# jwh97nn/AnyRef

Measured on AMD Instinct MI355X. Metric: images/sec (1024^2, 7B LLM+ViT-L+SAM-H), higher is better.
Workload: dtype bf16 (LLaMA / CLIP) + f16 (SAM encoder); 1 GPU; C2: LLaVA-7B + CLIP ViT-L/14 + SAM-H refer-seg forward, 1024x1024, S=320 prompt, 10 new tokens, KV cache; batch_per_gpu=1, global_batch=1, parallelism=dp1, weights=random-init N(0,0.02^2) rounded to bf16

## Files before the change

### anyref_amd/_lib.py

```python
from __future__ import annotations

import ctypes as C
import os

import torch

HERE = os.path.dirname(os.path.abspath(__file__))
LIB_PATH = os.path.join(HERE, "libanyref_hip.so")

ABI_VERSION = 2
F32, BF16, F16 = 0, 1, 2
MODE_PARITY, MODE_PERF, MODE_PERF_FP8W, MODE_PARITY16, MODE_PERF_F16, MODE_PARITY16_F16 = 0, 1, 2, 3, 4, 5
MODE_PERF_INT4W = 6


class AnyrefConfig(C.Structure):
    _fields_ = [
        ("abi_version", C.c_int32), ("mode", C.c_int32),
        ("clip_image", C.c_int32), ("clip_patch", C.c_int32), ("clip_dim", C.c_int32),
        ("clip_heads", C.c_int32), ("clip_layers_run", C.c_int32), ("clip_mlp", C.c_int32),
        ("clip_eps", C.c_float),
        ("llm_vocab", C.c_int32), ("llm_dim", C.c_int32), ("llm_heads", C.c_int32),
        ("llm_layers", C.c_int32), ("llm_mlp", C.c_int32), ("llm_max_seq", C.c_int32),
        ("llm_rms_eps", C.c_float), ("llm_rope_theta", C.c_float),
# ... 22 lines not shown
                                   "norm_out", "slabs_out")] +
                [(n, _L) for n in ("sA", "sW", "sC", "sR", "sBias")] +
                [(n, C.c_int32) for n in ("M", "N", "K", "lda", "ldw", "ldc", "ldr", "norm_ld", "act", "c_f32",
                                          "swiglu_pairs", "slabs", "max_wg", "batch")] +
                [("alpha", _F), ("norm_eps", _F), ("norm_done", C.c_int32)])


class NormEx(C.Structure):
    _fields_ = ([(n, _P) for n in ("x", "gain", "bias", "y", "row_map", "fill_dst", "fill_rows", "fill_bias")] +
                [(n, C.c_int32) for n in ("M", "D", "ldx", "ldy", "rms", "y_f32", "act", "fill_ld", "fill_n", "fill_N",
                                          "fill_fallback")] +
                [("eps", _F), ("fill_done", C.c_int32)])


class AttnEx(C.Structure):
    _fields_ = ([(n, _P) for n in ("q", "k", "v", "o", "q_pos0", "kv_len", "q_len", "rel_h", "rel_w", "rel_p",
                                   "rel_tab_h", "rel_tab_w")] +
                [(n, _L) for n in ("q_bs", "q_rs", "q_hs", "k_bs", "k_rs", "k_hs", "v_bs", "v_rs", "v_hs", "o_bs", "o_rs",
                                   "o_hs", "rel_hs")] +
                [(n, C.c_int32) for n in ("B", "H", "Sq", "Sk", "hd", "causal", "kh", "kw", "rel_ld", "rel_tab_ld",
                                          "max_wg")] +
                [("scale", _F)])

SYMBOLS = {
    "anyref_create": (_I, [C.POINTER(AnyrefConfig), _I, C.POINTER(_P)]),
    "anyref_destroy": (None, [_P]),
    "anyref_last_error": (C.c_char_p, [_P]),
    "anyref_set_weight": (_I, [_P, C.c_char_p, _P, _I, _I, C.POINTER(_L), _I]),
    "anyref_finalize": (_I, [_P]),
    "anyref_generate": (_I, [_P, _P, _P, _P, _P, _P, _I, _I, _P, _P, _I, _P, _P, _I, _I, _P, _P, _P, _P, _L, _P,
                             _P, _P]),
    "anyref_forward_teacher": (_I, [_P, _P, _P, _P, _P, _P, _I, _I, _P, _P, _I, _P, _P, _P, _P, _P, _L, _P, _P,
                                    _P, _P]),
    "anyref_encode_images": (_I, [_P, _P, _P, _I, _P, _P]),
    "anyref_sam_encode": (_I, [_P, _P, _P, _I, _P]),
    "anyref_mask_decode": (_I, [_P, _P, _P, _P, _I, _P, _P, _P, _P, _P]),
    "anyref_llm_forward": (_I, [_P, _P, _P, _P, _I, _I, _P, _P, _P, _P]),
    "anyref_project_audio": (_I, [_P, _P, _P, _I, _P]),
    "anyref_audio_encode": (_I, [_P, _P, _P, _I, _P]),
    "anyref_seg_tail": (_I, [_P, _P, _P, _P, _P, _P, _I, _I, _I, _P, _I, _P, _P, _P, _P, _P, _L, _P, _P]),
    "anyref_set_seg_range": (_I, [_P, _I, _I]),
    "anyref_set_overlap": (_I, [_P, _I]),
    "anyref_set_early_tail": (_I, [_P, _I]),
    "anyref_set_extra_event": (_I, [_P, _P]),
    "anyref_set_graphs": (_I, [_P, _I]),
    "anyref_set_side_share": (_I, [_P, _I, _I]),
    "anyref_profile_enable": (_I, [_P, _I]),
    "anyref_profile_config": (_I, [_P, C.c_char_p, _I]),
    "anyref_profile_collect": (_I, [_P]),
    "anyref_profile_calibrate": (_I, [_P, _P, C.POINTER(C.c_double)]),
    "anyref_profile_read": (_I, [_P, _I, C.c_char_p, _I, C.POINTER(C.c_double), C.POINTER(_L),
                                C.POINTER(C.c_double), C.POINTER(C.c_double)]),
    "anyref_stamps_enable": (_I, [_P, _I]),
    "anyref_stamps_collect": (_I, [_P, C.POINTER(_L)]),
    "anyref_stamps_dropped": (_I, [_P, C.POINTER(_L)]),
    "anyref_stamps_read": (_I, [_P, _L, C.c_char_p, _I, C.POINTER(C.c_double), C.POINTER(C.c_double),
                               C.POINTER(C.c_double), C.POINTER(_I)]),
    "anyref_stamps_spread": (_I, [_P, _L, C.POINTER(C.c_double), C.POINTER(C.c_double), C.POINTER(C.c_double)]),
    "anyref_device_bytes": (_L, [_P]),
    "anyref_mode_name": (C.c_char_p, [_P]),
    "anyref_inexact_weights": (_I, [_P, C.POINTER(_L)]),
    "anyref_op_gemm": (_I, [_I, _P, _P, _P, _P, _P, _P, _P, _I, _I, _I, _I, _I]),
    "anyref_op_gemm_fp8": (_I, [_P, _P, _P, _P, _P, _P, _P, _I, _I, _I, _I, _I]),
    "anyref_op_quant_fp8": (_I, [_P, _P, _I, _I, _P, _P]),
    "anyref_op_gemv_fp8": (_I, [_P, _P, _P, _F, _P, _P, _P, _P, _P, _P, _I, _I, _I]),
    "anyref_op_quant_int4": (_I, [_P, _P, _I, _I, _P, _P]),
    "anyref_op_dequant_int4": (_I, [_P, _P, _P, _I, _I, _P]),
    "anyref_op_gemm_int4": (_I, [_P, _P, _P, _P, _P, _P, _P, _I, _I, _I, _I, _I, _I]),
    "anyref_op_gemv_int4": (_I, [_P, _P, _P, _F, _P, _P, _P, _P, _P, _P, _I, _I, _I]),
    "anyref_op_iou_counts": (_I, [_P, _P, _P, _I, _L, _P]),
    "anyref_op_avs_counts": (_I, [_P, _P, _P, _I, _L, _P, _I, _F, _P, _P]),
    "anyref_op_sam_preprocess": (_I, [_P, _P, _I, _I, _I, C.POINTER(C.c_float), C.POINTER(C.c_float), _P]),
    "anyref_op_pil_resample_u8": (_I, [_P, _P, _I, _I, _I, _P, _P, _I, _I, _P, _P, _I, _P, _P, _I]),
    "anyref_op_pool_ref_tokens": (_I, [_P, _P, _I, _I, _I, _I, _P]),
    "anyref_op_kaldi_fbank": (_I, [_P, _P, _I, _I, _I, _I, _I, C.c_float, _P, _I, _P, _P, _I, C.c_float, C.c_float, _P]),
    "anyref_op_clip_finish": (_I, [_P, _P, _I, _I, _I, _I, _I, _I, _I, C.POINTER(C.c_float), C.POINTER(C.c_float), _P]),
    "anyref_op_gemv": (_I, [_I, _P, _P, _P, _F, _P, _P, _P, _P, _P, _I, _I, _I, _I]),
    "anyref_op_gemv_xn": (_I, [_I, _P, _P, _P, _F, _P, _P, _P, _P, _P, _I, _I, _I, _I, _P, _P, _I]),
    "anyref_op_split_roundtrip": (_I, [_I, _P, _P, _P, _P, _I, _I]),
    "anyref_op_rope_table": (_I, [_I, _I, _F, _P]),
    "anyref_op_decode_attn": (_I, [_I, _P, _P, _I, _I, _I, _P, _P, _P, _P, _I, _F, _P, _P, _I]),
    "anyref_op_rope_cache": (_I, [_I, _P, _P, _P, _P, _I, _I, _I, _I, _P, _P, _P, _P, _P, _P, _I, _P]),
    "anyref_op_argmax": (_I, [_P, _P, _I, _I, _I, _P, _P, _P, _I, _I, _I, _P, _P, _P]),
    "anyref_op_norm": (_I, [_I, _P, _P, _P, _P, _P, _I, _I, _F, _I]),
    "anyref_op_attention": (_I, [_I, _P, _P, _P, _P, _P, _I, _I, _I, _I, _I, _F, _I, _P, _P, _P, _I, _I]),
    "anyref_op_attention_tab": (_I, [_I, _P, _P, _P, _P, _P, _I, _I, _I, _I, _F, _P, _P, _I, _I, _I]),
    "anyref_op_gemm_gather": (_I, [_I, _P, _P, _P, _P, _P, _P, _P, _I, _I, _I, _I]),
    "anyref_op_attention_relp": (_I, [_I, _P, _P, _P, _P, _P, _I, _I, _I, _I, _F, _P, _I, _I, _I]),
    "anyref_op_rel_pos": (_I, [_I, _P, _P, _P, _P, _I, _I, _I, _I, _P, _P]),
    "anyref_op_postprocess": (_I, [_P, _P, _I, _I, _I, _I, _I, _I, _I, _I, _P]),
    "anyref_op_last_error": (C.c_char_p, []),
    "anyref_op_gemm_ex": (_I, [_I, _P, C.POINTER(GemmEx)]),
    "anyref_op_norm_ex": (_I, [_I, _P, C.POINTER(NormEx)]),
    "anyref_op_attention_ex": (_I, [_I, _P, C.POINTER(AttnEx)]),
    "anyref_op_last_tags": (C.c_char_p, []),
}

_lib = None


def load() -> C.CDLL:
    global _lib
    if _lib is not None:
        return _lib
    if not os.path.exists(LIB_PATH):
        raise RuntimeError(
            f"{LIB_PATH} not found: build the HIP backend first "
            "(`python -c 'import __graft_entry__ as g; g.build()'` or `make -C anyref_amd/csrc`). "
            "anyref_amd has no CPU fallback.")
    lib = C.CDLL(LIB_PATH)
    for name, (res, args) in SYMBOLS.items():
        fn = getattr(lib, name)
        fn.restype = res
        fn.argtypes = args
    _lib = lib
    return lib
```

### anyref_amd/csrc/common.h

```cpp
#pragma once
#include <hip/hip_runtime.h>
#include <stdint.h>
#include <atomic>
#include <stdio.h>
#include <stdexcept>

namespace anyref {

struct bf16 {
  uint16_t x;
};

__host__ __device__ inline float bf2f(bf16 h) {
  uint32_t u = ((uint32_t)h.x) << 16;
  return __builtin_bit_cast(float, u);
}
__device__ inline bf16 f2bf(float f) {
  __bf16 h = (__bf16)f;
  bf16 r;
  r.x = __builtin_bit_cast(uint16_t, h);
  return r;
}
inline bf16 f2bf_host(float f) {
  uint32_t u = __builtin_bit_cast(uint32_t, f);
// ... 207 lines not shown
  }
};
template <>
struct Vec16<float> {
  static constexpr int N = 4;
  static __device__ inline void unpack(const uint4v& v, float* f) {
#pragma unroll
    for (int i = 0; i < 4; ++i) {
      const uint32_t u = v[i];
      f[i] = __builtin_bit_cast(float, u);
    }
  }
};

typedef __attribute__((ext_vector_type(4))) short short4v_;
typedef __attribute__((ext_vector_type(8))) _Float16 half8v;
typedef __attribute__((ext_vector_type(4))) _Float16 half4v;
template <typename T>
__device__ __forceinline__ float4v mfma_16x16x32(short8 a, short8 b, float4v c) {
  if constexpr (is_half16<T>::value)
    return __builtin_amdgcn_mfma_f32_16x16x32_f16(__builtin_bit_cast(half8v, a), __builtin_bit_cast(half8v, b), c, 0, 0, 0);
  else
    return __builtin_amdgcn_mfma_f32_16x16x32_bf16(a, b, c, 0, 0, 0);
}
template <typename T>
__device__ __forceinline__ float4v mfma_16x16x16(short4v_ a, short4v_ b, float4v c) {
  if constexpr (is_half16<T>::value)
    return __builtin_amdgcn_mfma_f32_16x16x16f16(__builtin_bit_cast(half4v, a), __builtin_bit_cast(half4v, b), c, 0, 0, 0);
  else
    return __builtin_amdgcn_mfma_f32_16x16x16bf16_1k(a, b, c, 0, 0, 0);
}

typedef float float2v __attribute__((ext_vector_type(2)));
__device__ inline void unpack_fp8x16(const uint4v& v, float* f) {
#pragma unroll
  for (int i = 0; i < 4; ++i) {
    const int w = (int)v[i];
    const float2v lo = __builtin_amdgcn_cvt_pk_f32_fp8(w, false);
    const float2v hi = __builtin_amdgcn_cvt_pk_f32_fp8(w, true);
    f[4 * i] = lo[0]; f[4 * i + 1] = lo[1]; f[4 * i + 2] = hi[0]; f[4 * i + 3] = hi[1];
  }
}
constexpr float FP8_E4M3_MAX = 448.f;

enum Act : int { ACT_NONE = 0, ACT_RELU = 1, ACT_GELU = 2, ACT_QUICK_GELU = 3, ACT_SILU = 4 };

__device__ inline float apply_act(float v, int act) {
  switch (act) {
    case ACT_RELU:
      return v > 0.f ? v : 0.f;
    case ACT_GELU:
      return 0.5f * v * (1.f + erff(v * 0.70710678118654752f));
    case ACT_QUICK_GELU:
      return v / (1.f + __expf(-1.702f * v));
    case ACT_SILU:
      return v / (1.f + __expf(-v));
    default:
      return v;
  }
}

__device__ inline float gelu_fast(float v) {
  const float x = fabsf(v) * 0.70710678118654752f;
  const float t = __builtin_amdgcn_rcpf(fmaf(0.3275911f, x, 1.f));
  float p = fmaf(1.061405429f, t, -1.453152027f);
  p = fmaf(p, t, 1.421413741f);
  p = fmaf(p, t, -0.284496736f);
  p = fmaf(p, t, 0.254829592f);
  const float e = 1.f - p * t * __expf(-x * x);
  return 0.5f * v * (1.f + copysignf(e, v));
}

__device__ inline float wave_sum(float v) {
#pragma unroll
  for (int o = 32; o > 0; o >>= 1) v += __shfl_xor(v, o, 64);
  return v;
}
__device__ inline float wave_max(float v) {
#pragma unroll
  for (int o = 32; o > 0; o >>= 1) v = fmaxf(v, __shfl_xor(v, o, 64));
  return v;
}

#define HIP_TRY(expr)                                                                   \
  do {                                                                                  \
    hipError_t _e = (expr);                                                             \
    if (_e != hipSuccess) {                                                             \
      char _b[512];                                                                     \
      snprintf(_b, sizeof(_b), "%s failed: %s (%s:%d)", #expr, hipGetErrorString(_e), __FILE__, \
               __LINE__);                                                               \
      throw std::runtime_error(_b);                                                     \
    }                                                                                   \
  } while (0)

struct KernelAttrOnce {
  std::atomic<uint64_t> done[4] = {};
};
inline void ensure_dyn_lds(KernelAttrOnce& st, const void* kernel, int bytes) {
  int dev = 0;
  HIP_TRY(hipGetDevice(&dev));
  std::atomic<uint64_t>& word = st.done[(dev >> 6) & 3];
  const uint64_t bit = 1ull << (dev & 63);
  if (word.load(std::memory_order_acquire) & bit) return;
  HIP_TRY(hipFuncSetAttribute(kernel, hipFuncAttributeMaxDynamicSharedMemorySize, bytes));
  word.fetch_or(bit, std::memory_order_release);
}
inline int device_cus() {
  static std::atomic<int> cache[256] = {};
  int dev = 0;
  HIP_TRY(hipGetDevice(&dev));
  std::atomic<int>& c = cache[dev & 255];
  int v = c.load(std::memory_order_relaxed);
  if (!v) {
    HIP_TRY(hipDeviceGetAttribute(&v, hipDeviceAttributeMultiprocessorCount, dev));
    c.store(v, std::memory_order_relaxed);
  }
  return v;
}

__host__ __device__ inline int cdiv(int a, int b) { return (a + b - 1) / b; }
inline int64_t cdiv64(int64_t a, int64_t b) { return (a + b - 1) / b; }
inline int round_up(int a, int b) { return cdiv(a, b) * b; }

}
```

### anyref_amd/csrc/gemv.hip

```cpp
#include <cstdlib>
#include <stdexcept>
#include <type_traits>

#include "gemv_common.h"

namespace anyref {

#ifndef ANYREF_GEMV_NO_DOT2
#define ANYREF_GEMV_NO_DOT2 0
#endif
constexpr bool NO_DOT2 = ANYREF_GEMV_NO_DOT2;
template <typename T, int NB, bool DUAL, int XPT, bool W8 = false, bool PAIR = false>
__global__ __launch_bounds__(512) void gemv_kernel(GemvArgs a, int b0, int nb) {
  static_assert(!W8 || std::is_same<T, bf16>::value, "fp8 weights go with bf16 activations");
  using WE = typename split_term<T>::type;
  using XE = std::conditional_t<is_split<T>::value, float, T>;
  using WT = std::conditional_t<W8, uint8_t, WE>;
  constexpr int VN = W8 ? 16 : Vec16<WE>::N;
  constexpr int R = DUAL ? 1 : 2;
  constexpr int RW = 2;
  constexpr int UNR = 4;
  constexpr bool DOT2 = (std::is_same<T, bf16>::value || is_half16<T>::value) && !W8 && !NO_DOT2;
  extern __shared__ __attribute__((aligned(16))) char smem[];
  XE* xs = reinterpret_cast<XE*>(smem);
  __shared__ float red[NB][8];
  __shared__ float red2[2][4][2][NB];
  const int tid = threadIdx.x, lane = tid & 63, wave = tid >> 6;
  const int K = a.K;
  __shared__ unsigned long long st_t[2];
  __shared__ unsigned st_cnt;
  const unsigned long long t_begin = gemv_stamp_begin(a.stamp, st_t, st_cnt, tid);

  const WT* __restrict__ W = reinterpret_cast<const WT*>(a.W);
  const WT* __restrict__ W2 = reinterpret_cast<const WT*>(a.W2);
  const int ldw = a.ldw > 0 ? a.ldw : K;
  constexpr int CH = 64 * VN * UNR;
  const GemvWork<R, PAIR> wk(gridDim.x, blockIdx.x, wave, a.N, cdiv(K, CH));
  const int items = wk.items;
  uint4v wcur[UNR][RW], wnxt[UNR][RW];
  auto load_item = [&](int t, uint4v (&w)[UNR][RW]) {
    const auto it = wk.item(t);
    const int n0 = it.g * R;
#pragma unroll
    for (int u = 0; u < UNR; ++u) {
      const int k = it.live ? it.c * CH + u * 64 * VN + lane * VN : K;
#pragma unroll
      for (int r = 0; r < R; ++r) {
        const int n = n0 + r < a.N ? n0 + r : a.N - 1;
        w[u][r] = k < K ? __builtin_nontemporal_load(reinterpret_cast<const uint4v*>(W + (int64_t)n * ldw + k))
                        : uint4v{0, 0, 0, 0};
      }
      if (DUAL)
        w[u][RW - 1] = k < K ? __builtin_nontemporal_load(reinterpret_cast<const uint4v*>(W2 + (int64_t)n0 * ldw + k))
                             : uint4v{0, 0, 0, 0};
    }
  };
  if (!a.gain) {
    constexpr int XV = (XPT + 3) / 4;
    float4v xv[NB][XV];
#pragma unroll
    for (int b = 0; b < NB; ++b) {
      const float* x = a.x + (int64_t)(b0 + (b < nb ? b : 0)) * a.ldx;
#pragma unroll
      for (int i = 0; i < XV; ++i) {
        const int k = (tid + i * 512) * 4;
        xv[b][i] = (b < nb && k < K) ? *reinterpret_cast<const float4v*>(x + k) : float4v{0.f, 0.f, 0.f, 0.f};
      }
    }
    if (items > 0) load_item(0, wcur);
#pragma unroll
    for (int b = 0; b < NB; ++b) {
      if (b >= nb) continue;
#pragma unroll
      for (int i = 0; i < XV; ++i) {
        const int k = (tid + i * 512) * 4;
        if (k < K) store4_from_f32<XE>(&xs[b * K + k], xv[b][i][0], xv[b][i][1], xv[b][i][2], xv[b][i][3]);
      }
    }
  } else {
    constexpr int XV = (XPT + 3) / 4;
    GemvNormStage<NB, XV> st;
    st.load(a, b0, nb, tid);
    if (items > 0) load_item(0, wcur);
    float scale[NB];
    st.scales(a, red, lane, wave, scale);
#pragma unroll
    for (int b = 0; b < NB; ++b) {
      if (b >= nb) continue;
#pragma unroll
      for (int i = 0; i < XV; ++i) {
        const int k = (tid + i * 512) * 4;
        if (k < K) {
          const float4v v = st.xr[b][i] * scale[b] * st.gr[i];
          store4_from_f32<XE>(&xs[b * K + k], v[0], v[1], v[2], v[3]);
          gemv_store_xn(a, b0 + b, k, v);
        }
      }
    }
  }
  __syncthreads();

  float acc[RW][NB];
#pragma unroll
  for (int r = 0; r < RW; ++r)
#pragma unroll
    for (int b = 0; b < NB; ++b) acc[r][b] = 0.f;
  for (int t = 0; t < items; ++t) {
    if (t + 1 < items) load_item(t + 1, wnxt);
    const auto it = wk.item(t);
#pragma unroll
    for (int u = 0; u < UNR; ++u) {
      const int k = it.live ? it.c * CH + u * 64 * VN + lane * VN : K;
      if (k < K) {
        if constexpr (DOT2) {
          typedef __attribute__((ext_vector_type(2))) __bf16 bf16x2;
          typedef __attribute__((ext_vector_type(2))) _Float16 f16x2;
          uint4v xv[NB];
#pragma unroll
          for (int b = 0; b < NB; ++b)
            xv[b] = b < nb ? *reinterpret_cast<const uint4v*>(&xs[b * K + k]) : uint4v{0, 0, 0, 0};
#pragma unroll
          for (int r = 0; r < RW; ++r)
#pragma unroll
            for (int b = 0; b < NB; ++b)
#pragma unroll
              for (int j = 0; j < 4; ++j) {
                const uint32_t wj = wcur[u][r][j], xj = xv[b][j];
                if constexpr (is_half16<T>::value)
                  acc[r][b] = __builtin_amdgcn_fdot2(__builtin_bit_cast(f16x2, wj), __builtin_bit_cast(f16x2, xj), acc[r][b],
                                                     false);
                else
                  acc[r][b] = __builtin_amdgcn_fdot2_f32_bf16(__builtin_bit_cast(bf16x2, wj), __builtin_bit_cast(bf16x2, xj),
                                                              acc[r][b], false);
              }
        } else {
        float xf[NB][VN];
#pragma unroll
        for (int b = 0; b < NB; ++b) {
          if (b < nb) {
            constexpr int XV = Vec16<XE>::N;
#pragma unroll
            for (int h = 0; h < VN / XV; ++h) {
              const uint4v xv = *reinterpret_cast<const uint4v*>(&xs[b * K + k + h * XV]);
              Vec16<XE>::unpack(xv, &xf[b][h * XV]);
            }
          } else {
#pragma unroll
            for (int i = 0; i < VN; ++i) xf[b][i] = 0.f;
          }
        }
#pragma unroll
        for (int r = 0; r < RW; ++r) {
          float wf[VN];
          if constexpr (W8) unpack_fp8x16(wcur[u][r], wf);
          else Vec16<WE>::unpack(wcur[u][r], wf);
#pragma unroll
          for (int b = 0; b < NB; ++b)
#pragma unroll
            for (int i = 0; i < VN; ++i) acc[r][b] = fmaf(wf[i], xf[b][i], acc[r][b]);
        }
        }
      }
    }
    if (it.last) gemv_finish_group<NB, R, DUAL, W8, PAIR>(a, acc, red2, it.g, it.pass, wk.half, lane, wave, b0, nb);
    if (t + 1 < items) {
#pragma unroll
      for (int u = 0; u < UNR; ++u)
#pragma unroll
        for (int r = 0; r < RW; ++r) wcur[u][r] = wnxt[u][r];
    }
  }
  gemv_stamp_end(a.stamp, st_t, st_cnt, t_begin, lane);
}

template <bool W8, bool DUAL, int XV>
__global__ __launch_bounds__(512) void gemv_rows8_kernel(GemvArgs a, int b0, int nb, int kh0, int rs) {
  typedef __attribute__((ext_vector_type(2))) __bf16 bf16x2;
  constexpr int NB = 8, UNR = 8;
  constexpr int EPL = W8 ? 16 : 8;
  constexpr int SEG = 16 * EPL;
  constexpr int CH = UNR * SEG;
  using WT = std::conditional_t<W8, uint8_t, bf16>;
  extern __shared__ __attribute__((aligned(16))) char smem[];
  __shared__ float red[NB][8];
  const int tid = threadIdx.x, lane = tid & 63, wave = tid >> 6;
  const int j = lane & 3, q = lane >> 2;
  const int K = a.K;
  const int ldw = a.ldw > 0 ? a.ldw : K;
  const WT* __restrict__ W = reinterpret_cast<const WT*>(a.W);
  const WT* __restrict__ W2 = reinterpret_cast<const WT*>(a.W2);
  constexpr int R = DUAL ? 2 : 4;
  const int ngroups = cdiv(a.N, R);
  const int nwaves = gridDim.x * 8, gw = blockIdx.x * 8 + wave;
  const int my_groups = gw < ngroups ? (ngroups - gw + nwaves - 1) / nwaves : 0;
  const int nkh = kh0 < K ? 2 : 1;
  const int nch0 = cdiv(kh0, CH), nch1 = nkh == 2 ? cdiv(K - kh0, CH) : 0;
  const int items0 = my_groups * nch0, items = items0 + my_groups * nch1;
  const int pl = rs > 0 ? (rs - 64) / 2 : 0;
  uint4v w0[UNR], w1[UNR], w2[UNR];
  auto item_pos = [&](int t, int& g, int& kbeg, int& kend) __attribute__((always_inline)) {
    int gi, c;
    if (t < items0) {
      gi = t / nch0; c = t - gi * nch0;
      kbeg = c * CH; kend = kh0;
    } else {
      const int t1 = t - items0;
      gi = t1 / nch1; c = t1 - gi * nch1;
      kbeg = kh0 + c * CH; kend = K;
    }
    g = gw + gi * nwaves;
  };
  auto load_item = [&](int t, uint4v (&w)[UNR]) __attribute__((always_inline)) {
    int g, kbeg, kend;
    item_pos(t, g, kbeg, kend);
    const int jl = lane >> 4, ql = lane & 15;
    int n = DUAL ? g * 2 + (jl & 1) : g * 4 + jl;
    n = n < a.N ? n : a.N - 1;
    const WT* row = ((DUAL && jl >= 2) ? W2 : W) + (int64_t)n * ldw;
#pragma unroll
    for (int u = 0; u < UNR; ++u) {
      const int k = kbeg + u * SEG + ql * EPL;
      w[u] = k < kend ? __builtin_nontemporal_load(reinterpret_cast<const uint4v*>(row + k)) : uint4v{0, 0, 0, 0};
    }
  };
  auto xpos = [&](int b, int kl) __attribute__((always_inline)) {
    if constexpr (W8) return b * rs + ((kl >> 3) & 1) * pl + (kl >> 4) * 16 + (kl & 7) * 2;
    else return b * rs + kl * 2;
  };
  auto first_chunks = [&]() __attribute__((always_inline)) {
    if (items > 0) load_item(0, w0);
    if (items > 1) load_item(1, w1);
  };
  float scale[NB];
#pragma unroll
  for (int b = 0; b < NB; ++b) scale[b] = 1.f;
  if (a.gain) {
    GemvNormStage<NB, XV> st;
    st.load(a, b0, nb, tid);
    first_chunks();
    st.scales(a, red, lane, wave, scale);
#pragma unroll
    for (int b = 0; b < NB; ++b) {
#pragma unroll
      for (int i = 0; i < XV; ++i) {
        const int k = (tid + i * 512) * 4;
        if (k < K) {
          const float4v v = st.xr[b][i] * scale[b] * st.gr[i];
          store4_from_f32<bf16>(reinterpret_cast<bf16*>(smem + xpos(b, k)), v[0], v[1], v[2], v[3]);
          gemv_store_xn(a, b0 + b, k, v, b < nb);
        }
      }
    }
  }
  auto stage_plain = [&](int kbase, int klen, bool then_weights) __attribute__((always_inline)) {
// ... 119 lines not shown
    run(items0, items);
  }
}

static bool gemv_rows8_launch(const GemvArgs& a, int b0, int nb, hipStream_t s) {
  static const bool off = getenv("ANYREF_GEMV_ROWS8") && atoi(getenv("ANYREF_GEMV_ROWS8")) == 0;
  if (off) return false;
  const bool w8 = a.w_fp8 != 0, dual = a.W2 != nullptr;
  const int epl = w8 ? 16 : 8, ch = 8 * 16 * epl;
  const int ldw = a.ldw > 0 ? a.ldw : a.K;
  const size_t wsz = w8 ? 1 : 2;
  if (a.K % epl || (ldw * wsz) % 16 || ((uintptr_t)a.W & 15) || (dual && ((uintptr_t)a.W2 & 15)) || a.K % 4) return false;
  constexpr int KH_MAX = 9472;
  int kh0 = a.K;
  if (a.gain) {
    if (a.K > 6144) return false;
  } else if (a.K > KH_MAX) {
    kh0 = cdiv(cdiv(a.K, 2), ch) * ch;
    if (kh0 > KH_MAX || kh0 >= a.K) return false;
    if (cdiv(a.N, dual ? 2 : 4) > 256 * 8) return false;
  }
  const int rs = cdiv(kh0 * 2, 256) * 256 + 64;
  const size_t lds = (size_t)8 * rs;
  const int grid = 256;
  const double wbytes = (double)a.N * a.K * wsz * (dual ? 2 : 1) + (double)nb * (a.K + a.N) * 4;
  char tag[48];
  snprintf(tag, sizeof(tag), "gemv_rows8_%s%s", w8 ? "fp8w" : "bf16", dual ? "_swiglu" : "");
  ProfScope prof(tag, 2.0 * nb * a.N * (double)a.K * (dual ? 2 : 1), wbytes, s);
  auto launch = [&](auto w8_t, auto dual_t, auto xv_t) {
    gemv_launch<&gemv_rows8_kernel<decltype(w8_t)::value, decltype(dual_t)::value, decltype(xv_t)::value>, 152 * 1024>(
        grid, lds, s, a, b0, nb, kh0, rs);
  };
  using TT = std::true_type;
  using FF = std::false_type;
  using X2 = std::integral_constant<int, 2>;
  using X3 = std::integral_constant<int, 3>;
  auto by_xv = [&](auto w8_t, auto dual_t) {
    if (a.gain && a.K > 4096) launch(w8_t, dual_t, X3());
    else launch(w8_t, dual_t, X2());
  };
  if (w8) {
    if (dual) by_xv(TT(), TT());
    else by_xv(TT(), FF());
  } else {
    if (dual) by_xv(FF(), TT());
    else by_xv(FF(), FF());
  }
  return true;
}

template <typename T, int NB>
static void gemv_dispatch(const GemvArgs& a, int b0, int nb, hipStream_t s) {
  const size_t lds = (size_t)NB * a.K * (is_split<T>::value ? 4 : sizeof(T));
  const double wsz = a.w_fp8 ? 1.0 : (is_split<T>::value ? 2.0 : (double)sizeof(T));
  const double wbytes = (double)a.N * a.K * wsz * (a.W2 ? 2 : 1) + (double)nb * (a.K + a.N) * 4;
  const char* kind = a.w_fp8 ? "fp8w" : (is_split<T>::value ? (is_half16<typename split_term<T>::type>::value ? "sp16h" : "sp16") : is_half16<T>::value ? "f16" : sizeof(T) == 2 ? "bf16" : "f32");
  gemv_dispatch_pass("gemv", kind, a, lds, wbytes, nb, s, [&](auto xpt_t, auto dual_t, auto pair_t, const GemvArgs& g, int grid) {
    constexpr int XPT = decltype(xpt_t)::value;
    constexpr bool DUAL = decltype(dual_t)::value, PAIR = decltype(pair_t)::value;
    if constexpr (std::is_same<T, bf16>::value) {
      if (g.w_fp8) {
        gemv_launch<&gemv_kernel<T, NB, DUAL, XPT, true, PAIR>>(grid, lds, s, g, b0, nb);
        return;
      }
    }
    gemv_launch<&gemv_kernel<T, NB, DUAL, XPT, false, PAIR>>(grid, lds, s, g, b0, nb);
  });
}

template <typename T>
void launch_gemv(const GemvArgs& a, hipStream_t s) {
  if (a.w_int4) {
    if (!std::is_same<T, bf16>::value) throw std::runtime_error("gemv: int4 weights need the bf16 mode");
    launch_gemv_int4(a, s);
    return;
  }
  const int VN = a.w_fp8 ? 16 : Vec16<typename split_term<T>::type>::N;
  if (a.K % VN || ((uintptr_t)a.W & 15)) throw std::runtime_error("gemv: K must be a multiple of 16 bytes");
  if (a.w_fp8 && (!std::is_same<T, bf16>::value || !a.wscale || (a.W2 && !a.wscale2)))
    throw std::runtime_error("gemv: fp8 weights need the bf16 mode and per-row scales");
  if (((uintptr_t)a.x & 15) || a.ldx % 4 || a.K % 4 || (a.gain && ((uintptr_t)a.gain & 15)) ||
      (a.xn_out && (((uintptr_t)a.xn_out & 15) || a.xn_ld % 4)))
    throw std::runtime_error("gemv: x / gain / xn_out rows must be 16-byte aligned");
  int b0 = 0;
  if constexpr (std::is_same<T, bf16>::value) {
    while (a.B - b0 > 4) {
      const int n8 = a.B - b0 < 8 ? a.B - b0 : 8;
      if (!gemv_rows8_launch(a, b0, n8, s)) break;
      b0 += n8;
    }
  }
  gemv_passes<sizeof(T) == 2 ? 4 : 2>(b0, a.B, [&](auto nb_t, int p0, int nb) { gemv_dispatch<T, decltype(nb_t)::value>(a, p0, nb, s); });
}
template void launch_gemv<float>(const GemvArgs&, hipStream_t);

void launch_gemv_skinny_f32(const GemvArgs& a, hipStream_t s) {
  if (a.B < 1 || a.B > 8 || a.K > 4096 || a.K % 4 || a.W2 || a.w_fp8 || a.gain || ((uintptr_t)a.W & 15) ||
      ((uintptr_t)a.x & 15) || a.ldx % 4)
    throw std::runtime_error("gemv_skinny_f32: 1..8 rows, K <= 4096, K % 4 == 0, 16-byte aligned rows");
  const int ngroups = cdiv(a.N, 2);
  const int grid = ngroups >= 2048 ? 512 : cdiv(ngroups, 4);
  auto go = [&](auto nb_tag) {
    constexpr int NB = decltype(nb_tag)::value;
    ProfScope prof("gemv_f32_skinny", 2.0 * a.B * a.N * (double)a.K, (double)a.N * a.K * 4 + (double)a.B * (a.K + a.N) * 4,
                   s);
    gemv_launch<&gemv_kernel<float, NB, false, 8, false, true>>(grid, (size_t)NB * a.K * sizeof(float), s, a, 0, a.B);
  };
  if (a.B == 1) go(std::integral_constant<int, 1>());
  else if (a.B == 2) go(std::integral_constant<int, 2>());
  else if (a.B <= 4) go(std::integral_constant<int, 4>());
  else go(std::integral_constant<int, 8>());
}
template void launch_gemv<bf16>(const GemvArgs&, hipStream_t);
template void launch_gemv<sp16>(const GemvArgs&, hipStream_t);
template void launch_gemv<sp16h>(const GemvArgs&, hipStream_t);
template void launch_gemv<f16>(const GemvArgs&, hipStream_t);

}
```

### anyref_amd/csrc/gemv_common.h

```cpp
#pragma once
#include <cstdlib>
#include <stdexcept>
#include <string>
#include <type_traits>

#include "kernels.h"

namespace anyref {

template <int R, bool PAIR>
struct GemvWork {
  int ngroups, nch, unit, nunits, half, nchp, items;
  __device__ __forceinline__ GemvWork(unsigned grid, unsigned block, int wave, int N, int nch_) {
    const int nwaves = grid * 8, gw = block * 8 + wave;
    ngroups = cdiv(N, R);
    nch = nch_;
    unit = PAIR ? gw >> 1 : gw;
    nunits = PAIR ? nwaves >> 1 : nwaves;
    half = PAIR ? (gw & 1) : 0;
    nchp = PAIR ? (nch + 1) >> 1 : nch;
    const int my_groups = PAIR ? cdiv(ngroups, nunits) : (gw < ngroups ? (ngroups - gw + nwaves - 1) / nwaves : 0);
    items = my_groups * nchp;
  }
  struct Item {
    int pass, g, c;
    bool live, last;
  };
  __device__ __forceinline__ Item item(int t) const {
    const int pass = t / nchp, ci = t % nchp;
    const int g = unit + pass * nunits, c = PAIR ? 2 * ci + half : ci;
    return {pass, g, c, !PAIR || (g < ngroups && c < nch), ci == nchp - 1};
  }
};

template <int NB, int XV>
struct GemvNormStage {
  float4v xr[NB][XV], gr[XV];
  __device__ __forceinline__ void load_gain(const GemvArgs& a, int tid) {
#pragma unroll
    for (int i = 0; i < XV; ++i) {
      const int k = (tid + i * 512) * 4;
      gr[i] = k < a.K ? *reinterpret_cast<const float4v*>(a.gain + k) : float4v{1.f, 1.f, 1.f, 1.f};
    }
  }
  __device__ __forceinline__ void load_x(const GemvArgs& a, int b0, int nb, int tid) {
#pragma unroll
    for (int b = 0; b < NB; ++b) {
      const float* x = a.x + (int64_t)(b0 + (b < nb ? b : 0)) * a.ldx;
#pragma unroll
      for (int i = 0; i < XV; ++i) {
        const int k = (tid + i * 512) * 4;
        xr[b][i] = (b < nb && k < a.K) ? *reinterpret_cast<const float4v*>(x + k) : float4v{0.f, 0.f, 0.f, 0.f};
      }
    }
  }
  __device__ __forceinline__ void load(const GemvArgs& a, int b0, int nb, int tid) {
    load_gain(a, tid);
    load_x(a, b0, nb, tid);
  }
  __device__ __forceinline__ void scales(const GemvArgs& a, float (&red)[NB][8], int lane, int wave, float (&scale)[NB]) const {
#pragma unroll
    for (int b = 0; b < NB; ++b) {
      float ss = 0.f;
#pragma unroll
      for (int i = 0; i < XV; ++i)
#pragma unroll
        for (int e = 0; e < 4; ++e) ss += xr[b][i][e] * xr[b][i][e];
      ss = wave_sum(ss);
      if (lane == 0) red[b][wave] = ss;
    }
    __syncthreads();
#pragma unroll
    for (int b = 0; b < NB; ++b) {
      float tot = 0.f;
#pragma unroll
      for (int w = 0; w < 8; ++w) tot += red[b][w];
      scale[b] = rsqrtf(tot / (float)a.K + a.eps);
    }
  }
};
__device__ __forceinline__ void gemv_store_xn(const GemvArgs& a, int row, int k, float4v v, bool also = true) {
  if (a.xn_out && blockIdx.x == 0 && also)
    *reinterpret_cast<float4v*>(a.xn_out + (int64_t)(a.xn_row_map ? a.xn_row_map[row] : row) * a.xn_ld + k) = v;
}

template <bool DUAL, bool W8>
__device__ __forceinline__ void gemv_epilogue(const GemvArgs& a, float v, float v2, int n, int row) {
  if constexpr (W8) {
    v *= a.wscale[(int64_t)n * a.ws_stride];
    if (DUAL) v2 *= a.wscale2[(int64_t)n * a.ws_stride];
  }
  if (a.bias) v += a.bias[n];
  if (DUAL)
    v = apply_act(v, ACT_SILU) * v2;
  else
    v = apply_act(v, a.act);
  const int64_t o = (int64_t)row * a.ldy + n;
  if (a.resid) v += a.resid[o];
  a.y[o] = v;
}

template <int NB, int R, bool DUAL, bool W8, bool PAIR>
__device__ __forceinline__ void gemv_finish_group(const GemvArgs& a, float (&acc)[2][NB], float (&red2)[2][4][2][NB], int g,
                                                  int pass, int half, int lane, int wave, int b0, int nb) {
  constexpr int RW = 2;
  const int n0 = g * R;
#pragma unroll
  for (int r = 0; r < RW; ++r)
#pragma unroll
    for (int b = 0; b < NB; ++b) acc[r][b] = wave_sum(acc[r][b]);
  if constexpr (PAIR) {
    const int buf = pass & 1;
    if (half == 1 && lane == 0) {
#pragma unroll
      for (int r = 0; r < RW; ++r)
#pragma unroll
        for (int b = 0; b < NB; ++b) red2[buf][wave >> 1][r][b] = acc[r][b];
    }
    __syncthreads();
    if (half == 0) {
#pragma unroll
      for (int r = 0; r < RW; ++r)
#pragma unroll
        for (int b = 0; b < NB; ++b) acc[r][b] += red2[buf][wave >> 1][r][b];
    }
  }
  if (lane < R * NB && half == 0) {
    const int r = lane / NB, b = lane % NB, n = n0 + r;
    float v = 0.f, v2 = 0.f;
#pragma unroll
    for (int rr = 0; rr < R; ++rr)
#pragma unroll
      for (int bb = 0; bb < NB; ++bb)
        if (lane == rr * NB + bb) {
          v = acc[rr][bb];
          v2 = DUAL ? acc[RW - 1][bb] : 0.f;
        }
    if (n < a.N && b < nb) gemv_epilogue<DUAL, W8>(a, v, v2, n, b0 + b);
  }
#pragma unroll
  for (int r = 0; r < RW; ++r)
#pragma unroll
    for (int b = 0; b < NB; ++b) acc[r][b] = 0.f;
}

__device__ __forceinline__ unsigned long long gemv_stamp_begin(const StampArgs& st, unsigned long long (&st_t)[2],
                                                               unsigned& st_cnt, int tid) {
  unsigned long long t_begin = 0;
  if (st.base) {
    t_begin = wall_clock64();
    if (tid == 0) {
      st_t[0] = ~0ull;
      st_t[1] = 0;
      st_cnt = 0;
    }
  }
  return t_begin;
}
__device__ __forceinline__ void gemv_stamp_end(const StampArgs& st, unsigned long long (&st_t)[2], unsigned& st_cnt,
                                               unsigned long long t_begin, int lane) {
  if (st.base && lane == 0) {
    atomicMin(&st_t[0], t_begin);
    atomicMax(&st_t[1], (unsigned long long)wall_clock64());
    if (atomicAdd(&st_cnt, 1u) == 7u) {
      const int e = *st.epoch;
      if (e < st.max_epoch) {
        unsigned long long* p = st.base + (size_t)e * st.stride + (size_t)blockIdx.x * 2;
        p[0] = st_t[0];
        p[1] = st_t[1];
      }
    }
  }
}

inline bool gemv_pair_knob() {
  static const bool p = !(getenv("ANYREF_GEMV_PAIR") && atoi(getenv("ANYREF_GEMV_PAIR")) == 0);
  return p;
}
inline int gemv_grid_knob() {
  static const int g = getenv("ANYREF_GEMV_GRID") ? atoi(getenv("ANYREF_GEMV_GRID")) : 0;
  return g;
}

struct GemvPlan {
  int grid;
  bool pair;
};
inline GemvPlan gemv_plan(const GemvArgs& a, size_t lds) {
  const int grid_rule = 256 * (lds > 76 * 1024 ? 1 : 2);
  int grid = grid_rule;
  if (a.grid > 0 && a.grid < grid) grid = a.grid;
  if (gemv_grid_knob() > 0) grid = gemv_grid_knob();
  const bool pair = gemv_pair_knob() && cdiv(a.N, a.W2 ? 1 : 2) * 2 <= (gemv_grid_knob() > 0 ? grid : grid_rule) * 8;
  return {grid, pair};
}

template <auto KERN, int LDS_MAX = 150 * 1024, typename... Args>
inline void gemv_launch(int grid, size_t lds, hipStream_t s, Args... args) {
  static KernelAttrOnce once;
  ensure_dyn_lds(once, reinterpret_cast<const void*>(KERN), LDS_MAX);
  hipLaunchKernelGGL(KERN, dim3(grid), dim3(512), lds, s, args...);
}

template <typename Launch>
inline void gemv_dispatch_pass(const char* name, const char* kind, const GemvArgs& a_in, size_t lds, double wbytes, int nb,
                               hipStream_t s, Launch&& launch) {
  GemvArgs a = a_in;
  if (lds > 150 * 1024) throw std::runtime_error(std::string(name) + ": K too large for the LDS activation stage");
  const GemvPlan p = gemv_plan(a, lds);
  auto go = [&](auto xpt_t) {
    char tag[40];
    snprintf(tag, sizeof(tag), "gemv_%s%s_x%d", kind, a.W2 ? "_swiglu" : "", decltype(xpt_t)::value);
    ProfScope prof(tag, 2.0 * nb * a.N * (double)a.K * (a.W2 ? 2 : 1), wbytes, s);
    if (g_stamp && g_stamp->on) a.stamp = g_stamp->slot(tag, wbytes, p.grid);
    using TT = std::true_type;
    using FF = std::false_type;
    if (a.W2) {
      if (p.pair) launch(xpt_t, TT(), TT(), a, p.grid);
      else launch(xpt_t, TT(), FF(), a, p.grid);
    } else {
      if (p.pair) launch(xpt_t, FF(), TT(), a, p.grid);
      else launch(xpt_t, FF(), FF(), a, p.grid);
    }
  };
  if (a.K <= 512 * 8)
    go(std::integral_constant<int, 8>());
  else if (a.K <= 512 * 24)
    go(std::integral_constant<int, 24>());
  else if (a.K <= 512 * 32)
    go(std::integral_constant<int, 32>());
  else
    throw std::runtime_error(std::string(name) + ": K > 16384 not supported");
}

template <int NBMAX, typename Pass>
inline void gemv_passes(int b0, int B, Pass&& pass) {
  while (b0 < B) {
    const int left = B - b0, nb = left < NBMAX ? left : NBMAX;
    if (nb == 1)
      pass(std::integral_constant<int, 1>(), b0, nb);
    else if (nb == 2)
      pass(std::integral_constant<int, 2>(), b0, nb);
    else
      pass(std::integral_constant<int, NBMAX>(), b0, nb);
    b0 += nb;
  }
}

}
```

### anyref_amd/csrc/gemv_int4.hip

```cpp
#include <cstdlib>
#include <stdexcept>
#include <type_traits>

#include "gemv_common.h"

namespace anyref {

constexpr int I4_GROUP = 128;
constexpr int I4_BLOCK = 32;
constexpr float I4_BIAS = 136.f;

__global__ __launch_bounds__(256) void quant_int4_rows_kernel(const float* __restrict__ src, int lds, int K,
                                                              uint8_t* __restrict__ q, int ldq, bf16* __restrict__ scale,
                                                              int lds_scale, unsigned long long* __restrict__ inexact) {
  const int n = blockIdx.x, tid = threadIdx.x;
  const float* row = src + (int64_t)n * lds;
  uint32_t* out = reinterpret_cast<uint32_t*>(q + (int64_t)n * ldq);
  const int G = cdiv(K, I4_GROUP);
  unsigned changed = 0;
  for (int g0 = 0; g0 < G; g0 += 16) {
    const int g = g0 + (tid >> 4), k0 = g * I4_GROUP + (tid & 15) * 8;
    float w[8];
    float amax = 0.f;
#pragma unroll
// ... 76 lines not shown
  typedef __attribute__((ext_vector_type(2))) __bf16 bf16x2;
  constexpr int R = DUAL ? 1 : 2;
  constexpr int RW = 2;
  constexpr int UNR = XPT == 8 ? (PAIR ? 1 : 2) : XPT == 24 ? 3 : 4;
  constexpr int CHB = 64 * UNR;
  extern __shared__ __attribute__((aligned(16))) char smem[];
  __shared__ float red[NB][8];
  __shared__ float red2[2][4][2][NB];
  const int tid = threadIdx.x, lane = tid & 63, wave = tid >> 6;
  const int K = a.K, KB = cdiv(K, I4_BLOCK);
  const int row_bytes = KB * 64;
  float* xsum = reinterpret_cast<float*>(smem + (size_t)NB * row_bytes);
  __shared__ unsigned long long st_t[2];
  __shared__ unsigned st_cnt;
  const unsigned long long t_begin = gemv_stamp_begin(a.stamp, st_t, st_cnt, tid);

  const uint8_t* __restrict__ W = reinterpret_cast<const uint8_t*>(a.W);
  const uint8_t* __restrict__ W2 = reinterpret_cast<const uint8_t*>(a.W2);
  const uint16_t* __restrict__ S = reinterpret_cast<const uint16_t*>(a.gscale);
  const uint16_t* __restrict__ S2 = reinterpret_cast<const uint16_t*>(a.gscale2);
  const int ldw = a.ldw, lgs = a.ld_gscale;
  const GemvWork<R, PAIR> wk(gridDim.x, blockIdx.x, wave, a.N, cdiv(KB, CHB));
  const int items = wk.items;
  uint4v wcur[UNR][RW], wnxt[UNR][RW];
  uint32_t scur[UNR][RW], snxt[UNR][RW];
  auto load_item = [&](int t, uint4v (&w)[UNR][RW], uint32_t (&sc)[UNR][RW]) {
    const auto it = wk.item(t);
    const int n0 = it.g * R;
#pragma unroll
    for (int u = 0; u < UNR; ++u) {
      const int blk = it.live ? it.c * CHB + u * 64 + lane : KB;
#pragma unroll
      for (int r = 0; r < R; ++r) {
        const int n = n0 + r < a.N ? n0 + r : a.N - 1;
        w[u][r] = blk < KB ? __builtin_nontemporal_load(reinterpret_cast<const uint4v*>(W + (int64_t)n * ldw + blk * 16))
                           : uint4v{0, 0, 0, 0};
        sc[u][r] = blk < KB ? (uint32_t)S[(int64_t)n * lgs + (blk >> 2)] : 0u;
      }
      if (DUAL) {
        w[u][RW - 1] = blk < KB ? __builtin_nontemporal_load(reinterpret_cast<const uint4v*>(W2 + (int64_t)n0 * ldw + blk * 16))
                                : uint4v{0, 0, 0, 0};
        sc[u][RW - 1] = blk < KB ? (uint32_t)S2[(int64_t)n0 * lgs + (blk >> 2)] : 0u;
      }
    }
  };
  {
    constexpr int XV = (XPT + 3) / 4;
    GemvNormStage<NB, XV> st;
    if (a.gain) st.load_gain(a, tid);
    st.load_x(a, b0, nb, tid);
    if (items > 0) load_item(0, wcur, scur);
    float scale[NB];
#pragma unroll
    for (int b = 0; b < NB; ++b) scale[b] = 1.f;
    if (a.gain) st.scales(a, red, lane, wave, scale);
#pragma unroll
    for (int b = 0; b < NB; ++b) {
#pragma unroll
      for (int i = 0; i < XV; ++i) {
        const int k = (tid + i * 512) * 4;
        const float4v v = a.gain ? st.xr[b][i] * scale[b] * st.gr[i] : st.xr[b][i];
        const bf16 h0 = f2bf(v[0]), h1 = f2bf(v[1]), h2 = f2bf(v[2]), h3 = f2bf(v[3]);
        float sum = (bf2f(h0) + bf2f(h1)) + (bf2f(h2) + bf2f(h3));
        sum += __shfl_xor(sum, 1, 64);
        sum += __shfl_xor(sum, 2, 64);
        sum += __shfl_xor(sum, 4, 64);
        const int blk = k >> 5, in = k & 31;
        if (b < nb && blk < KB) {
          char* p = smem + (size_t)b * row_bytes + (size_t)(in >> 3) * (KB * 16) + blk * 16 + (in & 7) * 2;
          *reinterpret_cast<uint2v*>(p) = uint2v{(uint32_t)h0.x | ((uint32_t)h1.x << 16), (uint32_t)h2.x | ((uint32_t)h3.x << 16)};
          if ((tid & 7) == 0) xsum[b * KB + blk] = sum;
          if (a.gain) gemv_store_xn(a, b0 + b, k, v, k < K);
        }
      }
    }
  }
  __syncthreads();

  float acc[RW][NB];
#pragma unroll
  for (int r = 0; r < RW; ++r)
#pragma unroll
    for (int b = 0; b < NB; ++b) acc[r][b] = 0.f;
  for (int t = 0; t < items; ++t) {
    if (t + 1 < items) load_item(t + 1, wnxt, snxt);
    const auto it = wk.item(t);
#pragma unroll
    for (int u = 0; u < UNR; ++u) {
      const int blk = it.live ? it.c * CHB + u * 64 + lane : KB;
      if (blk < KB) {
        uint32_t pr[RW][16];
#pragma unroll
        for (int r = 0; r < RW; ++r)
#pragma unroll
          for (int d = 0; d < 4; ++d) {
            const uint32_t wd = wcur[u][r][d];
#pragma unroll
            for (int j = 0; j < 4; ++j) pr[r][d * 4 + j] = ((wd >> (4 * j)) & 0x000F000Fu) | 0x43004300u;
          }
        float sf[RW];
#pragma unroll
        for (int r = 0; r < RW; ++r) sf[r] = __builtin_bit_cast(float, scur[u][r] << 16);
#pragma unroll
        for (int b = 0; b < NB; ++b) {
          if (b >= nb) continue;
          const char* xb = smem + (size_t)b * row_bytes + blk * 16;
          uint4v xv[4];
#pragma unroll
          for (int d = 0; d < 4; ++d) xv[d] = *reinterpret_cast<const uint4v*>(xb + (size_t)d * (KB * 16));
          const float t0 = -I4_BIAS * xsum[b * KB + blk];
#pragma unroll
          for (int r = 0; r < RW; ++r) {
            float tt = t0;
#pragma unroll
            for (int d = 0; d < 4; ++d)
#pragma unroll
              for (int j = 0; j < 4; ++j) {
                const uint32_t xj = xv[d][j], pj = pr[r][d * 4 + j];
                tt = __builtin_amdgcn_fdot2_f32_bf16(__builtin_bit_cast(bf16x2, pj), __builtin_bit_cast(bf16x2, xj), tt, false);
              }
            acc[r][b] = fmaf(sf[r], tt, acc[r][b]);
          }
        }
      }
    }
    if (it.last) gemv_finish_group<NB, R, DUAL, false, PAIR>(a, acc, red2, it.g, it.pass, wk.half, lane, wave, b0, nb);
    if (t + 1 < items) {
#pragma unroll
      for (int u = 0; u < UNR; ++u)
#pragma unroll
        for (int r = 0; r < RW; ++r) {
          wcur[u][r] = wnxt[u][r];
          scur[u][r] = snxt[u][r];
        }
    }
  }
  gemv_stamp_end(a.stamp, st_t, st_cnt, t_begin, lane);
}

template <int NB>
static void gemv_int4_dispatch(const GemvArgs& a, int b0, int nb, hipStream_t s) {
  const int KB = cdiv(a.K, I4_BLOCK), G = cdiv(a.K, I4_GROUP);
  const size_t lds = (size_t)NB * KB * (64 + 4);
  const double wbytes = (double)a.N * ((double)a.K * 0.5 + G * 2.0) * (a.W2 ? 2 : 1) + (double)nb * (a.K + a.N) * 4;
  gemv_dispatch_pass("gemv_int4", "int4w", a, lds, wbytes, nb, s, [&](auto xpt_t, auto dual_t, auto pair_t, const GemvArgs& g, int grid) {
    gemv_launch<&gemv_int4_kernel<NB, decltype(dual_t)::value, decltype(xpt_t)::value, decltype(pair_t)::value>>(grid, lds, s, g, b0, nb);
  });
}

void launch_gemv_int4(const GemvArgs& a, hipStream_t s) {
  const int G = cdiv(a.K, I4_GROUP);
  if (a.K % 16 || ((uintptr_t)a.W & 15) || ((uintptr_t)a.W2 & 15) || a.ldw % 16 || a.ldw < G * 64)
    throw std::runtime_error("gemv_int4: K must be a multiple of 16 and nibble rows 16-byte aligned, whole groups long");
  if (!a.gscale || (a.W2 && !a.gscale2) || a.ld_gscale < G) throw std::runtime_error("gemv_int4: group scales missing");
  if (((uintptr_t)a.x & 15) || a.ldx % 4 || (a.gain && ((uintptr_t)a.gain & 15)) ||
      (a.xn_out && (((uintptr_t)a.xn_out & 15) || a.xn_ld % 4)))
    throw std::runtime_error("gemv_int4: x / gain / xn_out rows must be 16-byte aligned");
  gemv_passes<4>(0, a.B, [&](auto nb_t, int b0, int nb) { gemv_int4_dispatch<decltype(nb_t)::value>(a, b0, nb, s); });
}

}
```

### anyref_amd/csrc/kernels.h

```cpp
#pragma once
#include <cstdlib>
#include <map>
#include <string>
#include <utility>
#include <vector>

#include "common.h"

namespace anyref {

struct ProfStat {
  double ms = 0;
  int64_t count = 0;
  double flops = 0, bytes = 0;
};
class Profiler {
 public:
  ~Profiler();
  bool begin(const char* tag, double flops, double bytes, hipStream_t s);
  void end(hipStream_t s);
  void collect();
  void reset();
  void calibrate(hipStream_t s);
  double null_ms = 0.0;
// ... 56 lines not shown
  size_t cap_used_ = 0;
  int64_t dropped_ = 0;
  std::vector<Rec> eager_;
  std::map<int, std::vector<Rec>> graphs_;
  std::vector<int> epoch_keys_;
};
extern thread_local Stamper* g_stamp;
struct ProfScope {
  hipStream_t s;
  bool active;
  ProfScope(const char* tag, double flops, double bytes, hipStream_t st) : s(st), active(g_prof && g_prof->on) {
    if (active) active = g_prof->begin(tag, flops, bytes, s);
  }
  ~ProfScope() {
    if (active) g_prof->end(s);
  }
};

struct GemmArgs {
  const void* A = nullptr;
  const void* W = nullptr;
  const float* bias = nullptr;
  void* C = nullptr;
  const float* resid = nullptr;
  const int* row_map = nullptr;
  const int* a_row_map = nullptr;
  int M = 0, N = 0, K = 0;
  int lda = 0, ldw = 0, ldc = 0, ldr = 0;
  int act = ACT_NONE;
  int c_f32 = 0;
  float alpha = 1.f;
  int order = 3;
  int swiglu_pairs = 0;
  int w_fp8 = 0;
  const float* col_scale = nullptr;
  int w_int4 = 0;
  const void* gscale = nullptr;
  int ld_gscale = 0;
  int group_m = 0;
  int max_wg = 0;
  int vec_ok = 0;
  const float* norm_gain = nullptr;
  void* norm_out = nullptr;
  int norm_ld = 0;
  float norm_eps = 0.f;
  const float* norm_bias = nullptr;
  float* slabs_out = nullptr;
  int slabs = 0;
  bool* norm_done = nullptr;
  int batch = 1;
  int64_t sA = 0, sW = 0, sC = 0, sR = 0, sBias = 0;
};
template <typename T>
void launch_gemm(const GemmArgs& a, hipStream_t s);
void gemm_reserve_workspace(hipStream_t s, size_t bytes);
void gemm_release_workspace(hipStream_t s);
void attn_release_workspace(hipStream_t s);

struct GemvArgs {
  const float* x = nullptr;
  const float* gain = nullptr;
  float eps = 1e-6f;
  const void* W = nullptr;
  const void* W2 = nullptr;
  const float* bias = nullptr;
  float* y = nullptr;
  const float* resid = nullptr;
  int B = 1, N = 0, K = 0, ldx = 0, ldy = 0;
  int act = ACT_NONE;
  int ldw = 0;
  int w_fp8 = 0;
  const float* wscale = nullptr;
  const float* wscale2 = nullptr;
  int ws_stride = 1;
  int w_int4 = 0;
  const void* gscale = nullptr;
  const void* gscale2 = nullptr;
  int ld_gscale = 0;
  float* xn_out = nullptr;
  const int* xn_row_map = nullptr;
  int xn_ld = 0;
  StampArgs stamp;
  int grid = 0;
};
template <typename T>
void launch_gemv(const GemvArgs& a, hipStream_t s);
void launch_gemv_skinny_f32(const GemvArgs& a, hipStream_t s);
void launch_quant_fp8_rows(const float* src, int lds, int N, int K, uint8_t* q, int ldq, float* scale, hipStream_t s,
                           int scale_stride = 1, unsigned long long* inexact = nullptr);
void launch_dequant_fp8_rows(const uint8_t* q, int ldq, const float* scale, int N, int K, void* out_bf16, int ldo,
                             hipStream_t s);
void launch_quant_int4_rows(const float* src, int lds, int N, int K, uint8_t* q, int ldq, void* scale_bf16, int ld_scale,
                            hipStream_t s, unsigned long long* inexact = nullptr);
void launch_dequant_int4_rows(const uint8_t* q, int ldq, const void* scale_bf16, int ld_scale, int N, int K, void* out_bf16,
                              int ldo, hipStream_t s);
void launch_gemv_int4(const GemvArgs& a, hipStream_t s);

struct NormArgs {
  const float* x = nullptr;
  const float* gain = nullptr;
  const float* bias = nullptr;
  void* y = nullptr;
  const int* row_map = nullptr;
  int M = 0, D = 0, ldx = 0, ldy = 0;
  float eps = 1e-5f;
  int rms = 0;
  int y_f32 = 0;
  int act = ACT_NONE;
  void* fill_dst = nullptr;
  int fill_ld = 0, fill_n = 0, fill_N = 0;
  const int* fill_rows = nullptr;
  const float* fill_bias = nullptr;
  bool* fill_done = nullptr;
};
template <typename T>
void launch_norm(const NormArgs& a, hipStream_t s);

struct AttnArgs {
  const void *Q = nullptr, *K = nullptr, *V = nullptr;
  void* O = nullptr;
  int64_t q_bs = 0, q_rs = 0, q_hs = 0;
  int64_t k_bs = 0, k_rs = 0, k_hs = 0;
  int64_t v_bs = 0, v_rs = 0, v_hs = 0;
  int64_t o_bs = 0, o_rs = 0, o_hs = 0;
  int B = 0, H = 0, Sq = 0, Sk = 0, hd = 0;
  float scale = 1.f;
  int causal = 0;
  const int* q_pos0 = nullptr;
  const int* kv_len = nullptr;
  const int* q_len = nullptr;
  const float* rel_h = nullptr;
  const float* rel_w = nullptr;
  int kh = 0, kw = 0;
  const float* rel_p = nullptr;
  int64_t rel_hs = 0;
  int rel_ld = 0;
  const void* rel_tab_h = nullptr;
  const void* rel_tab_w = nullptr;
  int rel_tab_ld = 0;
  int o_f32 = 0;
  int o_split = 0;
  int sp16 = 0;
  int h_off = 0, h_total = 0;
  int max_wg = 0;
  int kv_splits = 1;
  float* part_o = nullptr;
  float* part_ml = nullptr;
};
template <typename T>
void launch_attention(const AttnArgs& a, hipStream_t s);
bool attention_takes_rel_tables(int elem_bytes, int hd, int Sq, int Sk, int kh, int kw, bool split = false);

template <typename T>
bool launch_decode_attn(const float* qkv, int B, int H, int hd, const int* pos, const float* cs_tab, void* kc,
                        void* vc, int maxS, float scale, float* out, void* q_keep, hipStream_t s);
template <typename T>
void launch_decode_step_attn(const float* qkv, int B, int H, int hd, const int* pos, const int* kv_len, const float* cs_tab,
                             void* q_tmp, void* kc, void* vc, int maxS, float scale, float* out, void* q_keep, hipStream_t s,
                             bool force_fallback = false);

template <typename T>
void launch_attn_row_mean(const void* q, int64_t q_bs, int64_t q_hs, const void* K, int64_t k_bs,
                          int64_t k_rs, int64_t k_hs, const int* kv_len, int B, int H, int hd,
                          float scale, float* out, int ld_out, hipStream_t s);

template <typename T>
void launch_rel_pos(const void* q, int64_t q_bs, int64_t q_rs, int64_t q_hs, const float* tab_h,
                    const float* tab_w, int B, int H, int size, int hd, float* rel_h, float* rel_w,
                    hipStream_t s);

template <typename T>
void launch_im2col_patch(const float* img, int B, int S, int p, void* out, int Kp, hipStream_t s);
template <typename T>
void launch_im2col_3x3(const void* in, int B, int g, int C, void* out, hipStream_t s);
template <typename T>
void launch_convert(const float* in, int64_t ld_in, void* out, int64_t ld_out, int rows, int cols,
                    hipStream_t s, unsigned long long* counts = nullptr);
void launch_unsplit(const void* in, int64_t ld_in, float* out, int64_t ld_out, int rows, int cols, hipStream_t s,
                    int f16_terms = 0);
void launch_add_rows(const float* a, const float* b, int bmod, float* out, int M, int D, hipStream_t s);
template <typename T>
void launch_add_rows_to(const float* a, const float* b, int bmod, void* out, int M, int D, hipStream_t s);
void launch_clip_assemble(const float* patch, const float* cls, const float* pos, float* x, int B, int n,
                          int D, hipStream_t s, int rows = 0);
template <typename T>
void launch_im2col_conv1(const float* img, int n, int Hh, int Ww, int k, int st, void* out, hipStream_t s);
void launch_l2norm_scale(const float* x, int rows, int D, float scale, float* y, hipStream_t s);
void launch_embed_splice(const int64_t* ids, const int* lens, int B, int Lmax, const void* emb_table,
                         int emb_dtype, int vocab, const float* img_feat, int n_img, float* x, int Smax,
                         int D, int* out_len, hipStream_t s);
void launch_scatter_rows(const float* rows, const int* dst_b, const int* dst_pos, int n, float* x, int Smax,
                         int D, hipStream_t s);
template <typename T>
void launch_rope_cache_slabs(const float* slab0, const float* slab1, int B, int S, int H, int hd, const int* pos0,
                             const int* lens, const float* cs_tab, void* q_out, void* kc, void* vc, int maxS, void* q_keep,
                             hipStream_t s);
template <typename T>
void launch_rope_cache(const void* qkv, int B, int S, int H, int hd, const int* pos0, const int* lens,
                       const float* cs_tab, void* q_out, void* kc, void* vc, int maxS, void* q_keep,
                       hipStream_t s);
template <typename T>
void launch_rope_cache_f32(const float* qkv, int B, int H, int hd, const int* pos, const float* cs_tab,
                           void* q_out, void* kc, void* vc, int maxS, void* q_keep, hipStream_t s);
void rope_table(int S, int hd, float theta, float* out);
void launch_embed_rows(const int64_t* ids, int B, const void* table, int dtype, int D, float* x, hipStream_t s);
void launch_decode_index(const int* pos, int B, int maxS, int* row_map, int* kvlen, hipStream_t s);
void launch_build_tokens(const float* out_tokens, int n_out, const float* pred, int n, int C, float* tokens,
                         hipStream_t s);
template <typename T>
void launch_swiglu(const void* gu, int M, int F, void* out, hipStream_t s);
void launch_argmax(const float* x, int M, int N, int ldx, int64_t* out, hipStream_t s, int* bump = nullptr);
void launch_argmax_next(const float* x, int M, int N, int ldx, int64_t* out, int* pos, const void* table, int dtype,
                        int D, int maxS, float* x_next, int* row_map, int* kvlen, hipStream_t s);
template <typename T>
void launch_upscale1(const float* tmp, int n, int g, int C, const float* ln_g, const float* ln_b, float eps,
                     void* out, hipStream_t s);
void launch_upscale2_masks(const float* tmp, const float* hyper, int n, int ntok, int g2, int C, float* masks,
                           hipStream_t s);
void launch_postprocess(const float* low, int64_t lstride, int n, int lh, int lw, int S, int rh, int rw, int H,
                        int W, float* out, hipStream_t s);
void launch_dense_pe(const float* gauss, int g, int F, float* out, hipStream_t s);
void launch_fill_i32(int* p, int v, int n, hipStream_t s);
void launch_add_i32(int* p, int v, int n, hipStream_t s);
template <typename T>
void launch_fill_rows_bias(void* dst, int ld, const int* rows, int nrows, const float* bias, int N, hipStream_t s);
void launch_iou_counts(const float* logits, const uint8_t* target, int n, int64_t hw, int64_t* counts, hipStream_t s);
void launch_avs_counts(const float* logits, const uint8_t* target, int n, int64_t hw, const float* cuts, int nth,
                       float cut_pred, int64_t* conf, int64_t* hist, hipStream_t s);
void launch_pool_ref_tokens(const float* f, int n, int L, int H, int n_out, float* out, hipStream_t s);
void launch_pil_resample_u8(const uint8_t* in, int H, int W, int C, uint8_t* tmp, uint8_t* out, int ow, int oh,
                            const int* xbounds, const int* xk, int kx, const int* ybounds, const int* yk, int ky,
                            hipStream_t s);
void launch_clip_finish(const uint8_t* img, int ih, int iw, int y0, int x0, int h, int w, int S, const float* mean,
                        const float* std_, float* out, hipStream_t s);
void launch_kaldi_fbank(const float* wave, int C, int T, int win, int shift, int padded, float preemph, const float* banks,
                        int n_mel, const double* tw, double* scratch, int target_len, float mean, float stdv, float* out,
                        hipStream_t s);
void launch_sam_preprocess(const uint8_t* img, int h, int w, int S, const float* mean, const float* std_, float* out,
                           hipStream_t s);
void launch_add_vec(const float* a, const float* v, float* out, int M, int D, hipStream_t s);
void launch_gather_rows(const float* x, int Smax, int D, const int* b, const int* pos, int n, float* out,
                        hipStream_t s);
void launch_rephrase(const float* hidden_b, int D, const float* attn_row, int s0, int e0, float weight,
                     float* y, hipStream_t s);
void launch_to_f32(const void* in, int dtype, float* out, int64_t n, hipStream_t s);



}
```

### anyref_amd/csrc/model.hip

```cpp
#include <algorithm>
#include <cmath>
#include <cstdlib>
#include <cstring>
#include <type_traits>

#include "model.h"

namespace anyref {

ModelBase::ModelBase(const anyref_config& c, int device) : cfg(c), device_(device) { HIP_TRY(hipSetDevice(device)); }

ModelBase::~ModelBase() {
  (void)hipSetDevice(device_);
  (void)hipDeviceSynchronize();
  for (auto& kv : allocs_) (void)hipFree(kv.first);
  if (wcount_) (void)hipFree(wcount_);
}

unsigned long long* ModelBase::weight_counts() {
  if (!wcount_) {
    HIP_TRY(hipMalloc(&wcount_, 2 * sizeof(unsigned long long)));
    HIP_TRY(hipMemset(wcount_, 0, 2 * sizeof(unsigned long long)));
  }
  return wcount_;
// ... 310 lines not shown
                           l.ng4 * rstride, 0, weight_counts());
  }
  Lin<W> alloc_int4(int n, int k, const std::string& name) {
    if (k % 16) throw std::runtime_error("int4 weights need K % 16 == 0: " + name + " has K = " + std::to_string(k));
    Lin<W> l;
    l.n = n;
    l.k = k;
    l.ng4 = cdiv(k, 128);
    l.ld4 = l.ng4 * 64 + kRowPadBytes;
    l.w4 = reinterpret_cast<uint8_t*>(dalloc((size_t)n * l.ld4));
    HIP_TRY(hipMemset(l.w4, 0x88, (size_t)n * l.ld4));
    l.s4 = talloc<bf16>((size_t)n * l.ng4);
    return l;
  }
  enum class WFmt { kInt4, kFp8 };
  Lin<W> alloc_quant(WFmt f, int n, int k, const std::string& name) {
    return f == WFmt::kInt4 ? alloc_int4(n, k, name) : alloc_fp8(n, k);
  }
  void pack_rows_quant(WFmt f, Lin<W>& l, int row0, const std::string& name, int rows, int cols, int rstride = 1) {
    if (f == WFmt::kInt4) pack_rows_int4(l, row0, name, rows, cols, rstride);
    else pack_rows_fp8(l, row0, name, rows, cols, rstride);
  }
  bool skinny_off_ = getenv("ANYREF_NO_SKINNY_GEMV") != nullptr;
  void gemmf(hipStream_t s, const float* A, int lda, const LinF& l, float* C, int ldc, int M, int act,
             const float* resid = nullptr, int ldr = 0) {
    if (M >= 1 && M <= 8 && l.k <= 4096 && l.k % 4 == 0 && lda % 4 == 0 && !((uintptr_t)A & 15) && (!resid || ldr == ldc) &&
        !skinny_off_) {
      GemvArgs g;
      g.x = A; g.ldx = lda; g.W = l.w; g.bias = l.b; g.y = C; g.ldy = ldc; g.resid = resid; g.B = M; g.N = l.n;
      g.K = l.k; g.act = act;
      launch_gemv_skinny_f32(g, s);
      return;
    }
    GemmArgs a;
    a.A = A; a.lda = lda; a.W = l.w; a.ldw = l.k; a.bias = l.b; a.C = C; a.ldc = ldc; a.M = M; a.N = l.n;
    a.K = l.k; a.act = act; a.c_f32 = 1; a.resid = resid; a.ldr = ldr;
    launch_gemm<float>(a, s);
  }
  template <typename E = T>
  void norm(hipStream_t s, const float* x, int ldx, const Affine& af, void* y, int ldy, int M, int D, float eps,
            bool y_f32, bool rms = false, const int* row_map = nullptr, int act = ACT_NONE) {
    NormArgs a;
    a.x = x; a.ldx = ldx; a.gain = af.g; a.bias = af.b; a.y = y; a.ldy = y_f32 ? ldy : apad<E>(ldy); a.M = M; a.D = D; a.eps = eps;
    a.rms = rms ? 1 : 0; a.y_f32 = y_f32 ? 1 : 0; a.row_map = row_map; a.act = act;
    launch_norm<E>(a, s);
  }

  void clip_tower(hipStream_t s, const float* images, int B);
  void llm_prefill(hipStream_t s, int B, int Sp, const int* lens_dev, bool keep_q);
  void llm_decode_step(hipStream_t s, int B, bool keep_q);
  void sam_encoder(hipStream_t s, const float* images, int B, float* out, int blk0 = 0, int blk1 = -1);
  void mask_decoder(hipStream_t s, const float* image_emb, const float* pred_emb, int n, float* masks4,
                    float* iou);
  void run_tail(hipStream_t s, const float* sam_images, int B, const std::vector<int>& seg_b,
                const std::vector<int>& seg_pos, const std::vector<int>& reph_s, const int32_t* resized_hw,
                const int32_t* orig_hw, int32_t* out_nseg, float* out_masks, int64_t out_masks_cap,
                int64_t* mask_offsets, float* out_low, const float* attn_given = nullptr, int attn_n = 0);
  void join_sam(hipStream_t s);
  void early_seg(hipEvent_t hidden_ready, int hidden_row, const int32_t* resized_hw, const int32_t* orig_hw,
                 float* out_masks, int64_t out_masks_cap, float* out_low);
  int early_done_ = 0;
  bool early_stop_ = false;
  void fork_sam(hipStream_t s, const float* sam_images, int B, bool fed = false);
  void sam_feed(int upto, bool capped);
  int cap_wg_ = 0;
  int sam_next_blk_ = 0;
  bool sam_enq_done_ = false;
  const float* sam_img_ = nullptr;
  int sam_B_ = 0;
  struct PendingEarly {
    hipEvent_t ready;
    int hidden_row;
    const int32_t *resized_hw, *orig_hw;
    float* out_masks;
    int64_t cap;
    float* out_low;
  };
  std::vector<PendingEarly> early_pending_;
  void early_seg_run(const PendingEarly& e);
  hipStream_t s2_ = nullptr;
  hipEvent_t ev_fork_ = nullptr, ev_sam_ = nullptr;
  bool sam_forked_ = false;
  void decode_step_graph(hipStream_t s, int B, bool keep_q, bool corun = false);
  hipStream_t cap_stream_ = nullptr;
  std::map<int, hipGraphExec_t> decode_graphs_;
  int splice_inputs(hipStream_t s, const int64_t* input_ids, const int32_t* lens, int B, int Lmax,
                    const float* extra_embeds, const int32_t* extra_slots, int n_extra,
                    std::vector<int>& slen, std::vector<int>& img_pos);
  void ensure_q_last();

  struct ClipLayer {
    Affine ln1, ln2;
    Lin<W> qkv, out, fc1, fc2;
  };
  int clip_n_ = 0, clip_kp_ = 0;
  Lin<W> clip_patch_;
  float *clip_cls_ = nullptr, *clip_pos_ = nullptr;
  Affine clip_pre_;
  std::vector<ClipLayer> clip_layers_;
  Lin<W> mm_proj_;
  T *c_col_ = nullptr, *c_h_ = nullptr, *c_att_ = nullptr, *c_mlp_ = nullptr, *c_feat_ = nullptr;
  Q* c_qkv_ = nullptr;
  float *c_patch_ = nullptr, *c_x_ = nullptr, *img_feat_ = nullptr;

  struct LlmLayer {
    Affine in_norm, post_norm;
    Lin<W> qkv, o, gu, down;
    W *gate_w = nullptr, *up_w = nullptr;
  };
  W* emb_table_ = nullptr;
  std::vector<LlmLayer> llm_layers_;
  Affine llm_norm_;
  Lin<W> lm_head_;
  float* rope_tab_ = nullptr;
  Q *kcache_ = nullptr, *vcache_ = nullptr, *q_last_ = nullptr;
  size_t cache_layer_stride_ = 0;
  float *l_x_ = nullptr, *hidden_all_ = nullptr, *l_logits_ = nullptr, *l_xlast_ = nullptr;
  T *l_h_ = nullptr, *l_att_ = nullptr, *l_act_ = nullptr;
  Q *l_qkv_ = nullptr, *l_q_ = nullptr;
  float *d_x_ = nullptr, *d_qkv_ = nullptr, *d_att_ = nullptr, *d_act_ = nullptr;
  Q* d_q_ = nullptr;
  int64_t *ids_dev_ = nullptr, *next_dev_ = nullptr;
  float* qkv_slabs_ = nullptr;
  bool qkv_slabs_off_ = getenv("ANYREF_NO_QKV_SLABS") != nullptr;
  int *lens_dev_ = nullptr, *slen_dev_ = nullptr, *pos_dev_ = nullptr, *kvlen_dev_ = nullptr, *rowmap_dev_ = nullptr,
      *idx_a_ = nullptr, *idx_b_ = nullptr;
  int64_t* next_host_ = nullptr;
  hipEvent_t ev_tok_[2] = {nullptr, nullptr};
  int* stage_ = nullptr;
  int *stage_first_ = nullptr, *stage_extra_ = nullptr, *stage_seg_ = nullptr, *stage_kl_ = nullptr;
  enum { ST_FIRST = 0, ST_EXTRA, ST_SEG, ST_KL, ST_N };
  hipEvent_t stage_ev_[ST_N] = {nullptr, nullptr, nullptr, nullptr};
  bool stage_busy_[ST_N] = {false, false, false, false};
  void stage_begin(int r) {
    if (stage_busy_[r]) HIP_TRY(hipEventSynchronize(stage_ev_[r]));
    stage_busy_[r] = false;
  }
  void stage_end(int r, hipStream_t s) {
    HIP_TRY(hipEventRecord(stage_ev_[r], s));
    stage_busy_[r] = true;
  }
  struct StageScope {
    Model* m;
    int r;
    hipStream_t s;
    StageScope(Model* m_, int r_, hipStream_t s_) : m(m_), r(r_), s(s_) { m->stage_begin(r); }
    ~StageScope() {
      try {
        m->stage_end(r, s);
      } catch (...) {
      }
    }
  };

  struct AudBlock {
    Affine ln1, ln2;
    Lin<W> qkv, out, fc1, fc2;
    float *bias_k = nullptr, *bias_v = nullptr;
  };
  std::vector<AudBlock> aud_blocks_;
  Lin<W> aud_stem_, aud_head_;
  Affine aud_stem_ln_, aud_head_ln_;
  float *aud_cls_ = nullptr, *aud_pos_ = nullptr, aud_scale_ = 20.f;
  int aud_np_ = 0, aud_rows_ = 0;
  int* aud_kvrow_ = nullptr;
  T *a_col_ = nullptr, *a_h_ = nullptr, *a_att_ = nullptr, *a_mlp_ = nullptr, *a_clsrow_ = nullptr;
  Q* a_qkv_ = nullptr;
  float *a_patch_ = nullptr, *a_x_ = nullptr, *a_emb_ = nullptr;

  LinF fc1_, fc2_;
  Lin<W> audio_proj_;
  bool has_audio_ = false;
  float *seg_h_ = nullptr, *seg_t_ = nullptr, *pred_emb_ = nullptr, *attn_row_ = nullptr;

  struct SamBlock {
    Affine ln1, ln2;
    Lin<WS> qkv, proj, lin1, lin2;
    Lin<QS> rel;
    bool global = false;
  };
  Lin<WS> sam_patch_;
  float* sam_pos_ = nullptr;
  std::vector<SamBlock> sam_blocks_;
  Lin<WS> neck0_, neck2_;
  Affine neck1_, neck3_;
  int sam_g_ = 0, sam_nw_ = 0, sam_wrows_ = 0;
  int *win2tok_ = nullptr, *tok2win_ = nullptr, *pad_rows_ = nullptr;
  int n_pad_rows_ = 0;
  TS *s_col_ = nullptr, *s_hglob_ = nullptr, *s_att_ = nullptr, *s_mlp_ = nullptr, *s_n1_ = nullptr, *s_col3_ = nullptr;
  QS* s_qkv_ = nullptr;
  float *s_x_ = nullptr, *s_relh_ = nullptr, *s_relw_ = nullptr, *s_n0_ = nullptr, *s_n2_ = nullptr,
        *sam_emb_ = nullptr;

  struct DecAttn {
    LinF q, k, v, o;
  };
  struct DecLayer {
    DecAttn self, t2i, i2t;
    Affine n1, n2, n3, n4;
    LinF lin1, lin2;
  };
  float *dense_pe_ = nullptr, *no_mask_ = nullptr, *out_tokens_ = nullptr;
  std::vector<DecLayer> dec_layers_;
  DecAttn dec_final_;
  Affine dec_norm_final_, up_ln_;
  LinF up1_, up2_;
  LinF hyper_[3], iou_head_[3];
  float *m_tokens_ = nullptr, *m_q_ = nullptr, *m_qp_ = nullptr, *m_keys_ = nullptr, *m_kp_ = nullptr,
        *m_qh_ = nullptr, *m_kh_ = nullptr, *m_vh_ = nullptr, *m_att_ = nullptr, *m_tmp_ = nullptr, *m_mlp_ = nullptr,
        *m_bigq_ = nullptr, *m_bigk_ = nullptr, *m_bigv_ = nullptr, *m_bigatt_ = nullptr, *m_up0_ = nullptr,
// ... 175 lines not shown
        pack_rows_quant(f, L.gu, 0, lp + "mlp.gate_proj.weight", F, H, 2);
        pack_rows_quant(f, L.gu, 1, lp + "mlp.up_proj.weight", F, H, 2);
        L.down = alloc_quant(f, H, F, lp + "mlp.down_proj.weight");
        pack_rows_quant(f, L.down, 0, lp + "mlp.down_proj.weight", H, F);
      } else {
        const int rp = kRowPadBytes / (int)sizeof(W), ldh = H + rp;
        L.qkv.n = 3 * H;
        L.qkv.k = H;
        L.qkv.ld = ldh;
        L.qkv.w = talloc<W>((size_t)3 * H * ldh);
        HIP_TRY(hipMemset(L.qkv.w, 0, (size_t)3 * H * ldh * sizeof(W)));
        for (int j = 0; j < 3; ++j) pack_rows(L.qkv.w, j * H, lp + "self_attn." + names[j] + ".weight", H, H, ldh);
        L.o = pack_linear(lp + "self_attn.o_proj.weight", "", H, H, 8, rp);
        L.gu.n = 2 * F;
        L.gu.k = H;
        L.gu.ld = ldh;
        L.gu.w = talloc<W>((size_t)2 * F * ldh);
        HIP_TRY(hipMemset(L.gu.w, 0, (size_t)2 * F * ldh * sizeof(W)));
        pack_rows(L.gu.w, 0, lp + "mlp.gate_proj.weight", F, H, 2 * ldh);
        pack_rows(L.gu.w + ldh, 0, lp + "mlp.up_proj.weight", F, H, 2 * ldh);
        L.gate_w = L.gu.w;
        L.up_w = L.gu.w + ldh;
        L.down = pack_linear(lp + "mlp.down_proj.weight", "", H, F, 8, rp);
        if (F % 8) throw std::runtime_error("llm_mlp must be a multiple of 8");
      }
      HIP_TRY(hipStreamSynchronize(0));
      for (const char* nm : {"self_attn.q_proj.weight", "self_attn.k_proj.weight", "self_attn.v_proj.weight",
                             "self_attn.o_proj.weight", "mlp.gate_proj.weight", "mlp.up_proj.weight",
                             "mlp.down_proj.weight"}) {
        auto it = raw_.find(lp + nm);
        if (it != raw_.end()) {
          dfree(it->second.p);
          raw_.erase(it);
        }
      }
    }
    llm_norm_ = affine("model.norm", false);
    if (fp8w_) {
      lm_head_ = alloc_fp8(V, H);
      pack_rows_fp8(lm_head_, 0, "lm_head.weight", V, H);
      const size_t big = std::max((size_t)2 * F * H, std::max((size_t)3 * H * H, (size_t)V * H));
      deq_buf_ = talloc<W>(big);
    } else {
      lm_head_ = pack_linear("lm_head.weight", "", V, H, 8, kRowPadBytes / (int)sizeof(W));
      if (int4w_) {
        size_t big = 0;
        if (H % 64) big = std::max((size_t)2 * F * H, (size_t)3 * H * H);
        if (F % 64) big = std::max(big, (size_t)H * F);
        if (big) deq_buf_ = talloc<W>(big);
      }
    }
    std::vector<float> tab((size_t)S * hd);
    rope_table(S, hd, c.llm_rope_theta, tab.data());
    rope_tab_ = upload_f32(tab);
    cache_layer_stride_ = (size_t)MB * S * H;
    kcache_ = talloc<Q>(cache_layer_stride_ * c.llm_layers);
    vcache_ = talloc<Q>(cache_layer_stride_ * c.llm_layers);
    const size_t R = (size_t)MB * S;
    l_x_ = talloc<float>(R * H);
    hidden_all_ = talloc<float>(R * H);
    l_h_ = aalloc<T>(R, std::max(H, c.audio_dim));
    l_qkv_ = talloc<Q>(R * 3 * H);
    if ((sizeof(T) == 2 || SPT) && (size_t)3 * H / 96 * 2 <= 256) qkv_slabs_ = talloc<float>((size_t)2 * 320 * 3 * H);
    l_q_ = talloc<Q>(R * H);
    l_att_ = aalloc<T>(R, H);
    l_act_ = aalloc<T>(R, F);
    l_logits_ = talloc<float>((size_t)MB * V);
    l_xlast_ = talloc<float>((size_t)MB * H);
    d_x_ = talloc<float>((size_t)MB * H);
    d_qkv_ = talloc<float>((size_t)MB * 3 * H);
    d_att_ = talloc<float>((size_t)MB * H);
    d_act_ = talloc<float>((size_t)MB * F);
    d_q_ = talloc<Q>((size_t)MB * H);
    ids_dev_ = talloc<int64_t>((size_t)MB * S);
    next_dev_ = talloc<int64_t>(MB);
    lens_dev_ = talloc<int>(MB);
    slen_dev_ = talloc<int>(MB);
    pos_dev_ = talloc<int>(MB);
    kvlen_dev_ = talloc<int>(MB);
    rowmap_dev_ = talloc<int>(MB);
    idx_a_ = talloc<int>((size_t)MB * std::max(c.max_seg, 64));
    idx_b_ = talloc<int>((size_t)MB * std::max(c.max_seg, 64));
    HIP_TRY(hipHostMalloc((void**)&next_host_, sizeof(int64_t) * MB * 2));
    for (auto& e : ev_tok_) HIP_TRY(hipEventCreateWithFlags(&e, hipEventDisableTiming));
    {
      const int n_first = 3 * MB, n_extra_max = 2 * MB * std::max(c.max_seg, 64), n_seg = 2 * MB * c.max_seg;
      HIP_TRY(hipHostMalloc((void**)&stage_, sizeof(int) * (size_t)(n_first + n_extra_max + n_seg + MB)));
      stage_first_ = stage_;
      stage_extra_ = stage_first_ + n_first;
      stage_seg_ = stage_extra_ + n_extra_max;
      stage_kl_ = stage_seg_ + n_seg;
      for (auto& e : stage_ev_) HIP_TRY(hipEventCreateWithFlags(&e, hipEventDisableTiming));
    }
    if (c.rephrase_weight > 0.f) ensure_q_last();
  }
  {
    const int H = c.llm_dim;
    fc1_ = pack_linear_f32("model.text_hidden_fcs.0.0.weight", "model.text_hidden_fcs.0.0.bias", H, H);
    fc2_ = pack_linear_f32("model.text_hidden_fcs.0.2.weight", "model.text_hidden_fcs.0.2.bias", c.out_dim, H);
    has_audio_ = has_raw("model.audio_projector.weight");
    if (has_audio_)
      audio_proj_ = pack_linear("model.audio_projector.weight", "model.audio_projector.bias", H, c.audio_dim);
    const size_t ns = (size_t)MB * c.max_seg;
    seg_h_ = talloc<float>(ns * H);
    seg_t_ = talloc<float>(ns * H);
    pred_emb_ = talloc<float>(ns * c.out_dim);
    attn_row_ = talloc<float>((size_t)MB * c.llm_max_seq);
  }
  {
    const std::string p = std::string(SAM_P) + "image_encoder.";
    const int D = c.sam_dim, g = c.sam_img / c.sam_patch, ws = c.sam_window, hd = D / c.sam_heads, C = c.sam_out_chans;
    const int nh_sam = c.sam_heads;
    sam_g_ = g;
    sam_nw_ = cdiv(g, ws);
    sam_wrows_ = sam_nw_ * sam_nw_ * ws * ws;
    if (SPS && (D % 64 || C % 64)) throw std::runtime_error("parity16: sam_dim / sam_out_chans must be multiples of 64");
    sam_patch_ = pack_linear<WS>(p + "patch_embed.proj.weight", p + "patch_embed.proj.bias", D, 3 * c.sam_patch * c.sam_patch);
    if (raw(p + "pos_embed").numel() != (int64_t)g * g * D) throw std::runtime_error("pos_embed shape mismatch");
    sam_pos_ = own_f32(p + "pos_embed");
    sam_blocks_.resize(c.sam_depth);
    for (int i = 0; i < c.sam_depth; ++i) {
      const std::string bp = p + "blocks." + std::to_string(i) + ".";
      SamBlock& L = sam_blocks_[i];
      for (int j = 0; j < c.sam_n_global; ++j)
        if (c.sam_global_idx[j] == i) L.global = true;
      L.ln1 = affine(bp + "norm1");
      L.ln2 = affine(bp + "norm2");
      L.qkv = pack_linear<WS>(bp + "attn.qkv.weight", bp + "attn.qkv.bias", 3 * D, D);
      L.proj = pack_linear<WS>(bp + "attn.proj.weight", bp + "attn.proj.bias", D, D);
      L.lin1 = pack_linear<WS>(bp + "mlp.lin1.weight", bp + "mlp.lin1.bias", c.sam_mlp_ratio * D, D);
      L.lin2 = pack_linear<WS>(bp + "mlp.lin2.weight", bp + "mlp.lin2.bias", D, c.sam_mlp_ratio * D);
      const int sz = L.global ? g : ws;
      resample_rel_pos(bp + "attn.rel_pos_h", 2 * sz - 1, hd);
      resample_rel_pos(bp + "attn.rel_pos_w", 2 * sz - 1, hd);
      const int Np = 2 * sz;
      const int kp = round_up(hd, 64) <= 3 * D - (nh_sam - 1) * hd ? round_up(hd, 64) : hd;
      L.rel.n = 2 * Np;
      L.rel.k = kp;
      L.rel.w = talloc<QS>((size_t)2 * Np * kp);
      HIP_TRY(hipMemset(L.rel.w, 0, (size_t)2 * Np * kp * sizeof(QS)));
      pack_rows(L.rel.w, 0, bp + "attn.rel_pos_h", 2 * sz - 1, hd, kp);
      pack_rows(L.rel.w, Np, bp + "attn.rel_pos_w", 2 * sz - 1, hd, kp);
    }
    neck0_ = pack_linear<WS>(p + "neck.0.weight", "", C, D);
    neck1_ = affine(p + "neck.1");
    neck3_ = affine(p + "neck.3");
    {
      std::vector<float> w = to_host(p + "neck.2.weight"), r((size_t)C * 9 * C);
      if (w.size() != r.size()) throw std::runtime_error("neck.2 shape mismatch");
      for (int o = 0; o < C; ++o)
        for (int ci = 0; ci < C; ++ci)
          for (int t = 0; t < 9; ++t) r[((size_t)o * 9 + t) * C + ci] = w[((size_t)o * C + ci) * 9 + t];
      float* rf = upload_f32(r);
      neck2_.n = C;
      neck2_.k = 9 * C;
      neck2_.w = talloc<WS>(r.size());
      launch_convert<WS>(rf, 9 * C, neck2_.w, 9 * C, C, 9 * C, 0, weight_counts());
      if constexpr (F16W) check_f16_range(p + "neck.2.weight");
      HIP_TRY(hipStreamSynchronize(0));
      dfree(rf);
    }
    std::vector<int> w2t((size_t)MB * sam_wrows_), t2w((size_t)MB * g * g);
    for (int b = 0; b < MB; ++b)
      for (int wy = 0; wy < sam_nw_; ++wy)
        for (int wx = 0; wx < sam_nw_; ++wx)
          for (int ty = 0; ty < ws; ++ty)
// ... 388 lines not shown
    Q* kc = kcache_ + cache_layer_stride_ * i;
    Q* vc = vcache_ + cache_layer_stride_ * i;
    if (!h_ready) norm(s, l_x_, H, L.in_norm, l_h_, H, R, H, c.llm_rms_eps, false, true);
    Q* qkeep = (keep_q && i == nl - 1) ? q_last_ : nullptr;
    if (qkv_slabs_ && !L.qkv.w8 && !L.qkv.w4 && R > 192 && R <= 320 && H % 128 == 0 && hd % 16 == 0 && !qkv_slabs_off_) {
      GemmArgs a;
      a.A = l_h_; a.lda = H; a.W = L.qkv.w; a.ldw = L.qkv.stride(); a.M = R; a.N = 3 * H; a.K = H;
      a.slabs_out = qkv_slabs_; a.slabs = 2;
      launch_gemm<T>(a, s);
      launch_rope_cache_slabs<Q>(qkv_slabs_, qkv_slabs_ + (size_t)R * 3 * H, B, Sp, nh, hd, nullptr, lens_dev, rope_tab_, l_q_,
                                 kc, vc, S, qkeep, s);
    } else {
      gemm(s, l_h_, H, L.qkv, l_qkv_, 3 * H, R, ACT_NONE, QF32);
      launch_rope_cache<Q>(l_qkv_, B, Sp, nh, hd, nullptr, lens_dev, rope_tab_, l_q_, kc, vc, S, qkeep, s);
    }
    AttnArgs a;
    a.Q = l_q_; a.K = kc; a.V = vc; a.O = l_att_;
    a.q_bs = (int64_t)Sp * H; a.q_rs = H; a.q_hs = hd;
    a.k_bs = a.v_bs = (int64_t)S * H; a.k_rs = a.v_rs = H; a.k_hs = a.v_hs = hd;
    a.o_bs = (int64_t)Sp * H; a.o_rs = H; a.o_hs = hd;
    a.B = B; a.H = nh; a.Sq = Sp; a.Sk = Sp; a.hd = hd;
    a.scale = 1.f / sqrtf((float)hd);
    a.causal = 1; a.kv_len = lens_dev; a.q_len = lens_dev;
    a.o_split = OSPT; a.sp16 = SPT;
    launch_attention<Q>(a, s);
    if (!gemm(s, l_att_, H, L.o, l_x_, H, R, ACT_NONE, true, l_x_, H, nullptr, &L.post_norm, l_h_))
      norm(s, l_x_, H, L.post_norm, l_h_, H, R, H, c.llm_rms_eps, false, true);
    gemm(s, l_h_, H, L.gu, l_act_, F, R, ACT_NONE, false, nullptr, 0, nullptr, nullptr, nullptr, true);
    h_ready = gemm(s, l_act_, F, L.down, l_x_, H, R, ACT_NONE, true, l_x_, H, nullptr,
                   i + 1 < nl ? &llm_layers_[i + 1].in_norm : nullptr, l_h_);
  }
  for (int b = 0; b < B; ++b)
    norm(s, l_x_ + (size_t)b * Sp * H, H, llm_norm_, hidden_all_ + (size_t)b * S * H, H, Sp, H, c.llm_rms_eps, true,
         true);
}

template <typename T, typename TS>
void Model<T, TS>::llm_decode_step(hipStream_t s, int B, bool keep_q) {
  const anyref_config& c = cfg;
  const int H = c.llm_dim, F = c.llm_mlp, nh = c.llm_heads, hd = H / nh, S = c.llm_max_seq, nl = c.llm_layers;
  static const bool rows8 = !(getenv("ANYREF_GEMV_ROWS8") && atoi(getenv("ANYREF_GEMV_ROWS8")) == 0);
  const bool mfma_decode = IS16 && B > ((std::is_same<T, bf16>::value && rows8) ? 8 : 4);
  bool h_ready = false;
  for (int i = 0; i < nl; ++i) {
    LlmLayer& L = llm_layers_[i];
    Q* kc = kcache_ + cache_layer_stride_ * i;
    Q* vc = vcache_ + cache_layer_stride_ * i;
    if (mfma_decode) {
      if (!h_ready) norm(s, d_x_, H, L.in_norm, l_h_, H, B, H, c.llm_rms_eps, false, true);
      gemm(s, l_h_, H, L.qkv, d_qkv_, 3 * H, B, ACT_NONE, true);
    } else {
      GemvArgs g;
      g.x = d_x_; g.ldx = H; g.gain = L.in_norm.g; g.eps = c.llm_rms_eps; gemv_w(g, L.qkv); g.y = d_qkv_;
      g.ldy = 3 * H; g.B = B; g.N = 3 * H; g.K = H;
      launch_gemv<T>(g, s);
    }
    Q* qk = (keep_q && i == nl - 1) ? q_last_ : nullptr;
    launch_decode_step_attn<Q>(d_qkv_, B, nh, hd, pos_dev_, kvlen_dev_, rope_tab_, d_q_, kc, vc, S, 1.f / sqrtf((float)hd),
                               d_att_, qk, s);
    if (mfma_decode) {
      launch_convert<T>(d_att_, H, l_att_, apad<T>(H), B, H, s);
      if (!gemm(s, l_att_, H, L.o, d_x_, H, B, ACT_NONE, true, d_x_, H, nullptr, &L.post_norm, l_h_))
        norm(s, d_x_, H, L.post_norm, l_h_, H, B, H, c.llm_rms_eps, false, true);
      gemm(s, l_h_, H, L.gu, l_act_, F, B, ACT_NONE, false, nullptr, 0, nullptr, nullptr, nullptr, true);
      h_ready = gemm(s, l_act_, F, L.down, d_x_, H, B, ACT_NONE, true, d_x_, H, nullptr,
                     i + 1 < nl ? &llm_layers_[i + 1].in_norm : nullptr, l_h_);
      continue;
    }
    GemvArgs o;
    o.x = d_att_; o.ldx = H; gemv_w(o, L.o); o.y = d_x_; o.resid = d_x_; o.ldy = H; o.B = B; o.N = H; o.K = H;
    launch_gemv<T>(o, s);
    GemvArgs m;
    m.x = d_x_; m.ldx = H; m.gain = L.post_norm.g; m.eps = c.llm_rms_eps; gemv_w(m, L.gu, 0, 2); gemv_w2(m, L.gu, 1);
    m.y = d_act_; m.ldy = F; m.B = B; m.N = F; m.K = H;
    launch_gemv<T>(m, s);
    GemvArgs d;
    d.x = d_act_; d.ldx = F; gemv_w(d, L.down); d.y = d_x_; d.resid = d_x_; d.ldy = H; d.B = B; d.N = H; d.K = F;
    launch_gemv<T>(d, s);
  }
  GemvArgs h;
  h.x = d_x_; h.ldx = H; h.gain = llm_norm_.g; h.eps = c.llm_rms_eps; gemv_w(h, lm_head_); h.y = l_logits_;
  h.ldy = c.llm_vocab; h.B = B; h.N = c.llm_vocab; h.K = H;
  h.xn_out = hidden_all_; h.xn_row_map = rowmap_dev_; h.xn_ld = H;
  launch_gemv<T>(h, s);
  launch_argmax_next(l_logits_, B, c.llm_vocab, c.llm_vocab, next_dev_, pos_dev_, emb_table_, kEmbDtype, H, S, d_x_,
                     rowmap_dev_, kvlen_dev_, s);
}

template <typename T, typename TS>
void Model<T, TS>::llm_forward(hipStream_t s, const float* embeds, const int32_t* lens, int B, int Sn, float* hidden,
                           float* logits, const int32_t* attn_q, float* attn_row) {
  HIP_TRY(hipSetDevice(device_));
  const anyref_config& c = cfg;
  if (B > c.max_batch || Sn > c.llm_max_seq) throw std::runtime_error("llm_forward: batch/seq exceed the model's limits");
  const int H = c.llm_dim;
  HIP_TRY(hipMemcpyAsync(l_x_, embeds, (size_t)B * Sn * H * 4, hipMemcpyDeviceToDevice, s));
  HIP_TRY(hipMemcpyAsync(lens_dev_, lens, B * 4, hipMemcpyHostToDevice, s));
  const bool keep_q = attn_q != nullptr;
  if (keep_q) ensure_q_last();
  llm_prefill(s, B, Sn, lens_dev_, keep_q);
  for (int b = 0; b < B; ++b)
    HIP_TRY(hipMemcpyAsync(hidden + (size_t)b * Sn * H, hidden_all_ + (size_t)b * c.llm_max_seq * H,
                           (size_t)Sn * H * 4, hipMemcpyDeviceToDevice, s));
  if (logits) {
    launch_convert<T>(hidden, H, l_h_, apad<T>(H), B * Sn, H, s);
    gemm(s, l_h_, H, lm_head_, logits, c.llm_vocab, B * Sn, ACT_NONE, true);
  }
  if (attn_q) {
    const int nh = c.llm_heads, hd = H / nh, S = c.llm_max_seq;
    std::vector<int> kl(B);
    for (int b = 0; b < B; ++b) kl[b] = attn_q[b] + 1;
    HIP_TRY(hipMemcpyAsync(kvlen_dev_, kl.data(), B * 4, hipMemcpyHostToDevice, s));
    HIP_TRY(hipStreamSynchronize(s));
    Q* kc = kcache_ + cache_layer_stride_ * (c.llm_layers - 1);
    for (int b = 0; b < B; ++b)
      launch_attn_row_mean<Q>(q_last_ + ((size_t)b * S + attn_q[b]) * H, 0, hd, kc + (size_t)b * S * H, 0, H, hd,
                              kvlen_dev_ + b, 1, nh, hd, 1.f / sqrtf((float)hd), attn_row + (size_t)b * Sn, Sn, s);
  }
}

template <typename T, typename TS>
void Model<T, TS>::sam_encoder(hipStream_t s, const float* images, int B, float* out, int blk0, int blk1) {
  const anyref_config& c = cfg;
  const int D = c.sam_dim, g = sam_g_, NT = g * g, RT = B * NT, ws = c.sam_window, nh = c.sam_heads, hd = D / nh;
  const int C = c.sam_out_chans, WR = sam_wrows_, nW = sam_nw_ * sam_nw_;
  const int nblk = (int)sam_blocks_.size();
  const bool to_end = blk1 < 0 || blk1 >= nblk;
  if (to_end) blk1 = nblk;
  static const bool per_image = getenv("ANYREF_SAM_PER_IMAGE") && atoi(getenv("ANYREF_SAM_PER_IMAGE")) != 0;
  if (B > 1 && per_image && blk0 == 0 && to_end) {
    for (int b = 0; b < B; ++b)
      sam_encoder(s, images + (size_t)b * 3 * c.sam_img * c.sam_img, 1, out + (size_t)b * NT * C, 0, -1);
    return;
  }
  if (blk0 == 0) {
    launch_im2col_patch<TS>(images, B, c.sam_img, c.sam_patch, s_col_, sam_patch_.k, s);
    GemmArgs a;
    a.A = s_col_; a.lda = sam_patch_.k; a.W = sam_patch_.w; a.ldw = sam_patch_.k; a.bias = sam_patch_.b;
    a.C = s_x_; a.ldc = D; a.M = NT; a.N = D; a.K = sam_patch_.k; a.c_f32 = 1;
    a.resid = sam_pos_; a.ldr = D;
    a.batch = B; a.sA = (int64_t)NT * sam_patch_.k; a.sC = (int64_t)NT * D; a.sR = 0;
    a.max_wg = cap_wg_;
    launch_gemm<TS>(a, s);
  }
  for (int bi = blk0; bi < blk1; ++bi) {
    auto& L = sam_blocks_[bi];
    AttnArgs a;
    a.max_wg = cap_wg_;
    a.q_hs = a.k_hs = a.v_hs = hd; a.o_hs = hd;
    a.q_rs = a.k_rs = a.v_rs = 3 * D; a.o_rs = D;
    a.H = nh; a.hd = hd; a.scale = 1.f / sqrtf((float)hd);
    a.Q = s_qkv_; a.K = s_qkv_ + D; a.V = s_qkv_ + 2 * D; a.O = s_att_;
    a.o_split = OSPS; a.sp16 = SPS;
    auto rel_gemm = [&](int rows) {
      GemmArgs r;
      r.A = s_qkv_; r.lda = 3 * D; r.sA = hd; r.W = L.rel.w; r.ldw = L.rel.k; r.sW = 0;
      r.C = s_relh_; r.ldc = L.rel.n; r.sC = (int64_t)rows * L.rel.n; r.M = rows; r.N = L.rel.n; r.K = L.rel.k;
      r.c_f32 = 1; r.batch = nh;
      launch_gemm<QS>(r, s);
      a.rel_p = s_relh_; a.rel_ld = L.rel.n; a.rel_hs = (int64_t)rows * L.rel.n;
    };
    if (L.global) {
      norm<TS>(s, s_x_, D, L.ln1, s_hglob_, D, RT, D, 1e-6f, false);
      gemm(s, s_hglob_, D, L.qkv, s_qkv_, 3 * D, RT, ACT_NONE, QF32S);
      rel_gemm(RT);
      a.q_bs = a.k_bs = a.v_bs = (int64_t)NT * 3 * D; a.o_bs = (int64_t)NT * D;
      a.B = B; a.Sq = NT; a.Sk = NT; a.kh = g; a.kw = g;
      launch_attention<QS>(a, s);
      gemm(s, s_att_, D, L.proj, s_x_, D, RT, ACT_NONE, true, s_x_, D);
// ... 287 lines not shown
  for (int i = 0; i < nseg; ++i) out_nseg[seg_b[i]]++;
  for (int b = 0; b < B; ++b)
    if (out_nseg[b] > c.max_seg) throw std::runtime_error("more [SEG] tokens in one image than max_seg");
  int64_t off = 0;
  for (int b = 0; b < B; ++b) {
    mask_offsets[b] = off;
    off += (int64_t)out_nseg[b] * orig_hw[2 * b] * orig_hw[2 * b + 1];
  }
  if (off > out_masks_cap) throw std::runtime_error("out_masks capacity too small");
  if (done > nseg) throw std::runtime_error("internal: more early [SEG] masks than [SEG] tokens");
  if (nseg == done) return;
  {
    StageScope stage_scope(this, ST_SEG, s);
    for (int i = 0; i < nseg; ++i) {
      stage_seg_[i] = seg_b[i];
      stage_seg_[nseg + i] = seg_pos[i];
    }
    HIP_TRY(hipMemcpyAsync(idx_a_, stage_seg_, nseg * 4, hipMemcpyHostToDevice, s));
    HIP_TRY(hipMemcpyAsync(idx_b_, stage_seg_ + nseg, nseg * 4, hipMemcpyHostToDevice, s));
  }
  launch_gather_rows(hidden_all_, S, H, idx_a_, idx_b_, nseg, seg_h_, s);
  if (c.rephrase_weight > 0.f) {
    StageScope stage_scope(this, ST_KL, s);
    const int nh = c.llm_heads, hd = H / nh;
    Q* kc = kcache_ + cache_layer_stride_ * (c.llm_layers - 1);
    std::vector<char> done(B, 0);
    for (int i = 0; i < nseg; ++i) {
      const int b = seg_b[i];
      if (done[b]) continue;
      done[b] = 1;
      const int e0 = seg_pos[i], s0 = reph_s[b];
      if (e0 <= s0) continue;
      if (attn_given) {
        HIP_TRY(hipMemcpyAsync(attn_row_ + (size_t)b * S, attn_given + ((size_t)b * attn_n + e0) * attn_n,
                               (size_t)attn_n * 4, hipMemcpyDeviceToDevice, s));
      } else {
        stage_kl_[b] = e0 + 1;
        HIP_TRY(hipMemcpyAsync(kvlen_dev_ + b, stage_kl_ + b, 4, hipMemcpyHostToDevice, s));
        launch_attn_row_mean<Q>(q_last_ + ((size_t)b * S + e0) * H, 0, hd, kc + (size_t)b * S * H, 0, H, hd,
                                kvlen_dev_ + b, 1, nh, hd, 1.f / sqrtf((float)hd), attn_row_ + (size_t)b * S, S, s);
      }
      launch_rephrase(hidden_all_ + (size_t)b * S * H, H, attn_row_ + (size_t)b * S, s0, e0, c.rephrase_weight,
                      seg_h_ + (size_t)i * H, s);
    }
  }
  gemmf(s, seg_h_, H, fc1_, seg_t_, H, nseg, ACT_RELU);
  gemmf(s, seg_t_, H, fc2_, pred_emb_, c.out_dim, nseg, ACT_NONE);
  if (!sam_ready) sam_encoder(s, sam_images, B, sam_emb_);
  const int NK = sam_g_ * sam_g_, C = c.sam_out_chans, L = 4 * sam_g_;
  int row = 0;
  for (int b = 0; b < B; ++b) {
    const int n = out_nseg[b];
    if (n == 0) continue;
    const int j0 = b == 0 ? done : 0;
    const int64_t hw = (int64_t)orig_hw[2 * b] * orig_hw[2 * b + 1];
    if (n > j0) {
      mask_decoder(s, sam_emb_ + (size_t)b * NK * C, pred_emb_ + (size_t)(row + j0) * c.out_dim, n - j0, nullptr, nullptr);
      launch_postprocess(m_masks_, (int64_t)c.num_mask_tokens * L * L, n - j0, L, L, c.sam_img, resized_hw[2 * b],
                         resized_hw[2 * b + 1], orig_hw[2 * b], orig_hw[2 * b + 1], out_masks + mask_offsets[b] + j0 * hw,
                         s);
      if (out_low)
        for (int j = j0; j < n; ++j)
          HIP_TRY(hipMemcpyAsync(out_low + ((size_t)b * c.max_seg + j) * L * L,
                                 m_masks_ + (size_t)(j - j0) * c.num_mask_tokens * L * L, (size_t)L * L * 4,
                                 hipMemcpyDeviceToDevice, s));
    }
    row += n;
  }
}

template <typename T, typename TS>
void Model<T, TS>::generate(hipStream_t s, const float* clip_images, const float* sam_images, const int64_t* input_ids,
                        const int32_t* lens, int B, int Lmax, const float* extra_embeds, const int32_t* extra_slots,
                        int n_extra, const int32_t* resized_hw, const int32_t* orig_hw, int max_new_tokens,
                        int eos_token_id, int64_t* out_ids, int32_t* out_lens, int32_t* out_nseg, float* out_masks,
                        int64_t out_masks_cap, int64_t* mask_offsets, float* out_low, float* out_hidden) {
  HIP_TRY(hipSetDevice(device_));
  const anyref_config& c = cfg;
  if (!finalized_) throw std::runtime_error("generate before finalize");
  if (B <= 0 || B > c.max_batch) throw std::runtime_error("batch exceeds max_batch");
  if (max_new_tokens < 1) throw std::runtime_error("max_new_tokens must be >= 1");
  const int H = c.llm_dim, S = c.llm_max_seq, n_img = clip_n_;
  const bool keep_q = c.rephrase_weight > 0.f;

  SamJoinGuard<Model<T, TS>> join_guard{this, s};
  const int nblk = (int)sam_blocks_.size();
  static const bool any_b = getenv("ANYREF_SIDE_ANYB") != nullptr;
  const int side_cap = B == 1 ? side_wgs_ : side_wgs_b_;
  const bool fed = (B <= 4 || any_b) && side_cap > 0 && overlap_ && IS16;
  const int steps_now = B == 1 ? side_steps_ : side_steps_b_;
  side_cap_now_ = side_cap;
  const int per_step = std::max(1, (nblk + steps_now - 1) / std::max(1, steps_now));
  if (fed) {
    fork_sam(s, sam_images, B, true);
    {
      static const int head_wgs = getenv("ANYREF_SIDE_HEAD_WGS") ? atoi(getenv("ANYREF_SIDE_HEAD_WGS")) : 0;
      if (head_wgs > 0) side_cap_now_ = head_wgs;
      sam_feed(std::min(side_head_, nblk - 1), true);
      side_cap_now_ = side_cap;
    }
  }
  clip_tower(s, clip_images, B);
  std::vector<int> slen, img_pos;
  if (extra_ev_) {
    hipEvent_t ev = reinterpret_cast<hipEvent_t>(extra_ev_);
    extra_ev_ = nullptr;
    HIP_TRY(hipStreamWaitEvent(s, ev, 0));
  }
  const int Sp = splice_inputs(s, input_ids, lens, B, Lmax, extra_embeds, extra_slots, n_extra, slen, img_pos);
  for (int b = 0; b < B; ++b)
    if (slen[b] + max_new_tokens > S) throw std::runtime_error("prompt + max_new_tokens exceeds llm_max_seq");
  {
    static const int pf_blocks = getenv("ANYREF_SIDE_PREFILL_BLOCKS") ? atoi(getenv("ANYREF_SIDE_PREFILL_BLOCKS")) : 0;
    if (fed && pf_blocks > 0) sam_feed(std::min(sam_next_blk_ + pf_blocks, nblk - 1), true);
  }
  llm_prefill(s, B, Sp, slen_dev_, keep_q);
  if (fed) {
    HIP_TRY(hipEventRecord(ev_fork_, s));
    HIP_TRY(hipStreamWaitEvent(s2_, ev_fork_, 0));
    sam_feed(sam_next_blk_ + per_step, true);
  } else {
    fork_sam(s, sam_images, B);
  }
  {
    {
    StageScope stage_scope(this, ST_FIRST, s);
    int *bb = stage_first_, *pp = stage_first_ + B, *sl = stage_first_ + 2 * B;
    for (int b = 0; b < B; ++b) {
      bb[b] = b;
      pp[b] = slen[b] - 1;
      sl[b] = slen[b] - 1;
    }
    HIP_TRY(hipMemcpyAsync(idx_a_, bb, B * 4, hipMemcpyHostToDevice, s));
    HIP_TRY(hipMemcpyAsync(idx_b_, pp, B * 4, hipMemcpyHostToDevice, s));
    HIP_TRY(hipMemcpyAsync(pos_dev_, sl, B * 4, hipMemcpyHostToDevice, s));
    }
    launch_gather_rows(hidden_all_, S, H, idx_a_, idx_b_, B, l_xlast_, s);
    GemvArgs h;
    h.x = l_xlast_; h.ldx = H; gemv_w(h, lm_head_); h.y = l_logits_; h.ldy = c.llm_vocab; h.B = B; h.N = c.llm_vocab;
    h.K = H;
    launch_gemv<T>(h, s);
    launch_argmax_next(l_logits_, B, c.llm_vocab, c.llm_vocab, next_dev_, pos_dev_, emb_table_, kEmbDtype, H, S, d_x_,
                       rowmap_dev_, kvlen_dev_, s);
  }
  std::vector<std::vector<int64_t>> gen(B);
  std::vector<char> fin(B, 0);
  const bool ahead = eos_token_id < 0;
  early_done_ = 0;
  early_stop_ = false;
  bool early = !early_off_ && sam_forked_ && B == 1 && c.rephrase_weight <= 0.f;
  for (int i = 1; early && i < lens[0]; ++i)
    if (input_ids[i] >= c.seg_lo && input_ids[i] <= c.seg_hi) early = false;
  int corun_tail = 1;
  auto corun_step = [&]() {
    if (!fed) return false;
    if (!sam_enq_done_) return true;
    return corun_tail-- > 0;
  };
  for (int step = 0; step < max_new_tokens; ++step) {
    int64_t* tok = next_host_ + (size_t)(step & 1) * c.max_batch;
    const bool last = step == max_new_tokens - 1;
    HIP_TRY(hipMemcpyAsync(tok, next_dev_, B * 8, hipMemcpyDeviceToHost, s));
    HIP_TRY(hipEventRecord(ev_tok_[step & 1], s));
    if (ahead && !last) {
      decode_step_graph(s, B, keep_q, corun_step());
      if (fed) sam_feed(sam_next_blk_ + per_step, true);
    }
    HIP_TRY(hipEventSynchronize(ev_tok_[step & 1]));
    bool all = true;
    for (int b = 0; b < B; ++b) {
      if (!fin[b]) {
        gen[b].push_back(tok[b]);
        if (eos_token_id >= 0 && tok[b] == eos_token_id) fin[b] = 1;
        if (early && !early_stop_ && tok[b] >= c.seg_lo && tok[b] <= c.seg_hi)
          early_seg(ev_tok_[step & 1], slen[0] + step - 1, resized_hw, orig_hw, out_masks, out_masks_cap, out_low);
      }
      all = all && fin[b];
    }
    if (all || last) break;
    if (!ahead) {
      decode_step_graph(s, B, keep_q, corun_step());
      if (fed) sam_feed(sam_next_blk_ + per_step, true);
    }
  }
  if (fed) sam_feed(nblk, false);
  const int Lout = Lmax + max_new_tokens;
  std::vector<int> seg_b, seg_pos, reph(B, 0);
  for (int b = 0; b < B; ++b) {
    int64_t* row = out_ids + (size_t)b * Lout;
    for (int i = 0; i < Lout; ++i) row[i] = 0;
    for (int i = 0; i < lens[b]; ++i) row[i] = input_ids[(size_t)b * Lmax + i];
    for (size_t i = 0; i < gen[b].size(); ++i) row[lens[b] + i] = gen[b][i];
    out_lens[b] = lens[b] + (int)gen[b].size();
    const int shift = img_pos[b] >= 0 ? n_img - 1 : 0;
    for (int p = 0; p + 1 < out_lens[b]; ++p) {
      const int64_t id = row[p + 1];
      if (id >= c.seg_lo && id <= c.seg_hi) {
        const int hp = p + shift;
        if (hp >= slen[b] + (int)gen[b].size() - 1) continue;
        seg_b.push_back(b);
        seg_pos.push_back(hp);
      }
    }
    reph[b] = lens[b] - 1 + shift;
  }
  run_tail(s, sam_images, B, seg_b, seg_pos, reph, resized_hw, orig_hw, out_nseg, out_masks, out_masks_cap,
           mask_offsets, out_low);
  if (out_hidden)
    HIP_TRY(hipMemcpyAsync(out_hidden, hidden_all_, (size_t)B * S * H * 4, hipMemcpyDeviceToDevice, s));
}

template <typename T, typename TS>
void Model<T, TS>::forward_teacher(hipStream_t s, const float* clip_images, const float* sam_images,
                               const int64_t* input_ids, const int32_t* lens, int B, int Lmax,
                               const float* extra_embeds, const int32_t* extra_slots, int n_extra,
                               const int32_t* rephrase_start, const int32_t* resized_hw, const int32_t* orig_hw,
                               int32_t* out_nseg, float* out_masks, int64_t out_masks_cap, int64_t* mask_offsets,
                               float* out_low, float* out_hidden, float* out_logits) {
  HIP_TRY(hipSetDevice(device_));
  const anyref_config& c = cfg;
  if (!finalized_) throw std::runtime_error("forward before finalize");
  if (B <= 0 || B > c.max_batch) throw std::runtime_error("batch exceeds max_batch");
  const int H = c.llm_dim, S = c.llm_max_seq, n_img = clip_n_;
  const bool keep_q = c.rephrase_weight > 0.f;
  early_done_ = 0;
  early_stop_ = false;
  SamJoinGuard<Model<T, TS>> join_guard{this, s};
  fork_sam(s, sam_images, B);
  clip_tower(s, clip_images, B);
  std::vector<int> slen, img_pos;
  if (extra_ev_) {
    hipEvent_t ev = reinterpret_cast<hipEvent_t>(extra_ev_);
    extra_ev_ = nullptr;
    HIP_TRY(hipStreamWaitEvent(s, ev, 0));
  }
  const int Sp = splice_inputs(s, input_ids, lens, B, Lmax, extra_embeds, extra_slots, n_extra, slen, img_pos);
  llm_prefill(s, B, Sp, slen_dev_, keep_q);
  if (out_logits) {
    for (int b = 0; b < B; ++b) {
      launch_convert<T>(hidden_all_ + (size_t)b * S * H, H, l_h_, apad<T>(H), slen[b], H, s);
      gemm(s, l_h_, H, lm_head_, out_logits + (size_t)b * Sp * c.llm_vocab, c.llm_vocab, slen[b], ACT_NONE, true);
    }
  }
  std::vector<int> seg_b, seg_pos, reph(B, 0);
  for (int b = 0; b < B; ++b) {
    const int shift = img_pos[b] >= 0 ? n_img - 1 : 0;
    for (int p = 1; p < lens[b]; ++p) {
      const int64_t id = input_ids[(size_t)b * Lmax + p];
      if (id >= c.seg_lo && id <= c.seg_hi) {
        seg_b.push_back(b);
        seg_pos.push_back(p - 1 + shift);
      }
    }
    reph[b] = rephrase_start ? rephrase_start[b] - 1 + shift : 0;
  }
  run_tail(s, sam_images, B, seg_b, seg_pos, reph, resized_hw, orig_hw, out_nseg, out_masks, out_masks_cap,
           mask_offsets, out_low);
// ... 54 lines not shown
```

### anyref_amd/csrc/ops.hip

```cpp
#include <algorithm>
#include <cstring>
#include <type_traits>

#include "kernels.h"

namespace anyref {

thread_local Profiler* g_prof = nullptr;

Profiler::~Profiler() {
  for (auto& p : pool_) {
    (void)hipEventDestroy(p.first);
    (void)hipEventDestroy(p.second);
  }
}
bool Profiler::begin(const char* tag, double flops, double bytes, hipStream_t s) {
  if (!filter.empty() && strncmp(tag, filter.c_str(), filter.size()) != 0) return false;
  int t = -1;
  for (size_t i = 0; i < tags_.size(); ++i)
    if (tags_[i] == tag) t = (int)i;
  if (t < 0) {
    tags_.push_back(tag);
    stats_.push_back(ProfStat());
    seen_.push_back(0);
// ... 873 lines not shown
template void launch_rope_cache<bf16>(const void*, int, int, int, int, const int*, const int*, const float*,
                                      void*, void*, void*, int, void*, hipStream_t);
template void launch_rope_cache<f16>(const void*, int, int, int, int, const int*, const int*, const float*,
                                     void*, void*, void*, int, void*, hipStream_t);
template <typename T>
void launch_rope_cache_f32(const float* qkv, int B, int H, int hd, const int* pos, const float* cs_tab,
                           void* q_out, void* kc, void* vc, int maxS, void* q_keep, hipStream_t s) {
  hipLaunchKernelGGL((rope_cache_kernel<T, float>), dim3(1, B), dim3(256), 0, s, qkv, B, 1, H, hd, pos, nullptr,
                     cs_tab, reinterpret_cast<T*>(q_out), reinterpret_cast<T*>(kc), reinterpret_cast<T*>(vc),
                     maxS, reinterpret_cast<T*>(q_keep));
}
void rope_table(int S, int hd, float theta, float* out) {
  for (int pos = 0; pos < S; ++pos)
    for (int d = 0; d < hd / 2; ++d) {
      const float inv = 1.0f / powf(theta, (float)(2 * d) / (float)hd);
      const float fr = (float)pos * inv;
      out[((size_t)pos * 2) * (hd / 2) + d] = cosf(fr);
      out[((size_t)pos * 2 + 1) * (hd / 2) + d] = sinf(fr);
    }
}
template void launch_rope_cache_f32<float>(const float*, int, int, int, const int*, const float*, void*, void*,
                                           void*, int, void*, hipStream_t);
template void launch_rope_cache_f32<bf16>(const float*, int, int, int, const int*, const float*, void*, void*,
                                          void*, int, void*, hipStream_t);
template void launch_rope_cache_f32<f16>(const float*, int, int, int, const int*, const float*, void*, void*,
                                         void*, int, void*, hipStream_t);

__global__ void embed_rows_kernel(const int64_t* __restrict__ ids, const void* __restrict__ table, int dtype,
                                  int D, float* __restrict__ x) {
  const int b = blockIdx.x;
  table_row_to_f32(table, dtype, ids[b], D, x + (int64_t)b * D, threadIdx.x, blockDim.x);
}
void launch_embed_rows(const int64_t* ids, int B, const void* table, int dtype, int D, float* x,
                       hipStream_t s) {
  hipLaunchKernelGGL(embed_rows_kernel, dim3(B), dim3(256), 0, s, ids, table, dtype, D, x);
}
__global__ void decode_index_kernel(const int* __restrict__ pos, int B, int maxS, int* __restrict__ row_map,
                                    int* __restrict__ kvlen) {
  const int b = threadIdx.x;
  if (b < B) {
    row_map[b] = b * maxS + pos[b];
    kvlen[b] = pos[b] + 1;
  }
}
void launch_decode_index(const int* pos, int B, int maxS, int* row_map, int* kvlen, hipStream_t s) {
  hipLaunchKernelGGL(decode_index_kernel, dim3(1), dim3(64), 0, s, pos, B, maxS, row_map, kvlen);
}
__global__ void build_tokens_kernel(const float* __restrict__ out_tokens, int n_out, const float* __restrict__ pred,
                                    int C, float* __restrict__ tokens) {
  const int i = blockIdx.y, t = blockIdx.x;
  const float* src = t < n_out ? out_tokens + (int64_t)t * C : pred + (int64_t)i * C;
  float* dst = tokens + ((int64_t)i * (n_out + 1) + t) * C;
  for (int d = threadIdx.x; d < C; d += blockDim.x) dst[d] = src[d];
}
void launch_build_tokens(const float* out_tokens, int n_out, const float* pred, int n, int C, float* tokens,
                         hipStream_t s) {
  if (n <= 0) return;
  hipLaunchKernelGGL(build_tokens_kernel, dim3(n_out + 1, n), dim3(256), 0, s, out_tokens, n_out, pred, C, tokens);
}

template <typename T>
__global__ void swiglu_kernel(const T* __restrict__ gu, int M, int F, T* __restrict__ out) {
  const int64_t total = (int64_t)M * F;
  for (int64_t i = blockIdx.x * (int64_t)blockDim.x + threadIdx.x; i < total;
       i += (int64_t)gridDim.x * blockDim.x) {
    const int64_t m = i / F;
    const int j = (int)(i % F);
    const float g = to_f32<T>(gu[m * 2 * F + j]), u = to_f32<T>(gu[m * 2 * F + F + j]);
    out[i] = from_f32<T>(apply_act(g, ACT_SILU) * u);
  }
}
template <typename T>
void launch_swiglu(const void* gu, int M, int F, void* out, hipStream_t s) {
  const int64_t total = (int64_t)M * F;
  if (total <= 0) return;
  const int grid = (int)(cdiv64(total, 256) < 8192 ? cdiv64(total, 256) : 8192);
  hipLaunchKernelGGL((swiglu_kernel<T>), dim3(grid), dim3(256), 0, s, reinterpret_cast<const T*>(gu), M, F,
                     reinterpret_cast<T*>(out));
}
template void launch_swiglu<float>(const void*, int, int, void*, hipStream_t);
template void launch_swiglu<bf16>(const void*, int, int, void*, hipStream_t);
template void launch_swiglu<f16>(const void*, int, int, void*, hipStream_t);

__device__ __forceinline__ void argmax_take(float v, int i, float& best, int& bi) {
  const bool vn = __builtin_isnan(v), bn = __builtin_isnan(best);
  if (vn || bn) {
    if (vn && (!bn || i < bi)) {
      best = v;
      bi = i;
    }
    return;
  }
  if (v > best || (v == best && i < bi)) {
    best = v;
    bi = i;
  }
}
struct ArgmaxNext {
  const void* table = nullptr;
  int dtype = 0, D = 0, maxS = 0;
  float* x = nullptr;
  int* row_map = nullptr;
  int* kvlen = nullptr;
};
__global__ __launch_bounds__(1024) void argmax_kernel(const float* __restrict__ x, int N, int ldx,
                                                      int64_t* __restrict__ out, int* __restrict__ bump,
                                                      ArgmaxNext nx) {
  constexpr int NT = 1024, U = 8;
  const float* row = x + (int64_t)blockIdx.x * ldx;
  const int tid = threadIdx.x, lane = tid & 63, wave = tid >> 6;
  float best = -INFINITY;
  int bi = 0x7fffffff;
  if ((ldx & 3) == 0 && ((uintptr_t)x & 15) == 0) {
    const int n4 = N >> 2;
    for (int i0 = 0; i0 < n4; i0 += NT * U) {
      float4 v[U];
#pragma unroll
      for (int u = 0; u < U; ++u) {
        const int i = i0 + u * NT + tid;
        v[u] = i < n4 ? reinterpret_cast<const float4*>(row)[i] : float4{-INFINITY, -INFINITY, -INFINITY, -INFINITY};
      }
#pragma unroll
      for (int u = 0; u < U; ++u) {
        const int i = (i0 + u * NT + tid) * 4;
        argmax_take(v[u].x, i, best, bi);
        argmax_take(v[u].y, i + 1, best, bi);
        argmax_take(v[u].z, i + 2, best, bi);
        argmax_take(v[u].w, i + 3, best, bi);
      }
    }
    for (int i = n4 * 4 + tid; i < N; i += NT) argmax_take(row[i], i, best, bi);
  } else {
    for (int i = tid; i < N; i += NT) argmax_take(row[i], i, best, bi);
  }
#pragma unroll
  for (int o = 32; o > 0; o >>= 1) {
    const float v = __shfl_xor(best, o, 64);
    const int i = __shfl_xor(bi, o, 64);
    argmax_take(v, i, best, bi);
  }
  __shared__ float sv[NT / 64];
  __shared__ int si[NT / 64];
  if (lane == 0) {
    sv[wave] = best;
    si[wave] = bi;
  }
  __syncthreads();
  if (tid == 0) {
    for (int w = 1; w < NT / 64; ++w) argmax_take(sv[w], si[w], best, bi);
    out[blockIdx.x] = bi;
    si[0] = bi;
    if (bump) {
      const int p = bump[blockIdx.x] + 1;
      bump[blockIdx.x] = p;
      if (nx.x) {
        nx.row_map[blockIdx.x] = blockIdx.x * nx.maxS + p;
        nx.kvlen[blockIdx.x] = p + 1;
      }
    }
  }
  if (!nx.x) return;
  __syncthreads();
  const int64_t id = si[0];
  float* dst = nx.x + (int64_t)blockIdx.x * nx.D;
  table_row_to_f32(nx.table, nx.dtype, id, nx.D, dst, tid, NT);
}
void launch_argmax(const float* x, int M, int N, int ldx, int64_t* out, hipStream_t s, int* bump) {
  if (M <= 0) return;
  hipLaunchKernelGGL(argmax_kernel, dim3(M), dim3(1024), 0, s, x, N, ldx, out, bump, ArgmaxNext{});
}
void launch_argmax_next(const float* x, int M, int N, int ldx, int64_t* out, int* pos, const void* table, int dtype,
                        int D, int maxS, float* x_next, int* row_map, int* kvlen, hipStream_t s) {
  if (M <= 0) return;
  ArgmaxNext nx;
  nx.table = table; nx.dtype = dtype; nx.D = D; nx.maxS = maxS; nx.x = x_next; nx.row_map = row_map; nx.kvlen = kvlen;
  hipLaunchKernelGGL(argmax_kernel, dim3(M), dim3(1024), 0, s, x, N, ldx, out, pos, nx);
}

template <typename T>
__global__ __launch_bounds__(256) void upscale1_kernel(const float* __restrict__ tmp, int n, int g, int C,
                                                       const float* __restrict__ ln_g,
                                                       const float* __restrict__ ln_b, float eps,
                                                       T* __restrict__ out) {
  const int lane = threadIdx.x & 63, wave = threadIdx.x >> 6;
  const int64_t pix = (int64_t)blockIdx.x * 4 + wave;
  const int G = 2 * g;
  if (pix >= (int64_t)n * G * G) return;
  const int X = (int)(pix % G), Y = (int)((pix / G) % G), i = (int)(pix / ((int64_t)G * G));
  const float* src = tmp + (((int64_t)i * g + Y / 2) * g + X / 2) * 4 * C + ((Y & 1) * 2 + (X & 1)) * C;
  float v0 = lane < C ? src[lane] : 0.f, v1 = lane + 64 < C ? src[lane + 64] : 0.f;
  const float mean = wave_sum(v0 + v1) / (float)C;
  const float c0 = lane < C ? v0 - mean : 0.f, c1 = lane + 64 < C ? v1 - mean : 0.f;
  const float var = wave_sum(c0 * c0 + c1 * c1) / (float)C;
  const float inv = 1.f / sqrtf(var + eps);
  T* dst = out + pix * C;
  if (lane < C) dst[lane] = from_f32<T>(apply_act(c0 * inv * ln_g[lane] + ln_b[lane], ACT_GELU));
  if (lane + 64 < C) dst[lane + 64] = from_f32<T>(apply_act(c1 * inv * ln_g[lane + 64] + ln_b[lane + 64], ACT_GELU));
}
template <typename T>
void launch_upscale1(const float* tmp, int n, int g, int C, const float* ln_g, const float* ln_b, float eps,
                     void* out, hipStream_t s) {
  if (C > 128) throw std::runtime_error("upscale1: C > 128");
  const int64_t pix = (int64_t)n * 4 * g * g;
  hipLaunchKernelGGL((upscale1_kernel<T>), dim3((unsigned)cdiv64(pix, 4)), dim3(256), 0, s, tmp, n, g, C, ln_g,
                     ln_b, eps, reinterpret_cast<T*>(out));
}
template void launch_upscale1<float>(const float*, int, int, int, const float*, const float*, float, void*,
                                     hipStream_t);
template void launch_upscale1<bf16>(const float*, int, int, int, const float*, const float*, float, void*,
                                    hipStream_t);

__global__ void upscale2_masks_kernel(const float* __restrict__ tmp, const float* __restrict__ hyper, int n,
                                      int ntok, int g2, int C, float* __restrict__ masks) {
  extern __shared__ float hs[];
  const int i = blockIdx.y;
  for (int j = threadIdx.x; j < ntok * C; j += blockDim.x) hs[j] = hyper[(int64_t)i * ntok * C + j];
  __syncthreads();
  const int G = 2 * g2;
  const int64_t pix = (int64_t)blockIdx.x * blockDim.x + threadIdx.x;
  if (pix >= (int64_t)G * G) return;
  const int X = (int)(pix % G), Y = (int)(pix / G);
  const float* src = tmp + (((int64_t)i * g2 + Y / 2) * g2 + X / 2) * 4 * C + ((Y & 1) * 2 + (X & 1)) * C;
  float acc[8];
#pragma unroll
  for (int t = 0; t < 8; ++t) acc[t] = 0.f;
  for (int c = 0; c < C; ++c) {
    const float u = apply_act(src[c], ACT_GELU);
#pragma unroll
    for (int t = 0; t < 8; ++t)
      if (t < ntok) acc[t] = fmaf(hs[t * C + c], u, acc[t]);
  }
  for (int t = 0; t < ntok; ++t) masks[(((int64_t)i * ntok + t) * G + Y) * G + X] = acc[t];
}
void launch_upscale2_masks(const float* tmp, const float* hyper, int n, int ntok, int g2, int C, float* masks,
                           hipStream_t s) {
  if (ntok > 8) throw std::runtime_error("upscale2: more than 8 mask tokens");
  const int G = 2 * g2;
  dim3 grid((unsigned)cdiv64((int64_t)G * G, 256), n);
  hipLaunchKernelGGL(upscale2_masks_kernel, grid, dim3(256), ntok * C * sizeof(float), s, tmp, hyper, n, ntok,
                     g2, C, masks);
}

__device__ inline void bil_idx(int dst, float scale, int in, int& i0, int& i1, float& l1) {
  float src = scale * ((float)dst + 0.5f) - 0.5f;
  if (src < 0.f) src = 0.f;
  i0 = (int)src;
  if (i0 > in - 1) i0 = in - 1;
  i1 = i0 < in - 1 ? i0 + 1 : i0;
  l1 = src - (float)i0;
}
__device__ inline float bil_stage1(const float* __restrict__ low, int lh, int lw, float sy, float sx, int y,
                                   int x) {
  int y0, y1, x0, x1;
  float ly, lx;
  bil_idx(y, sy, lh, y0, y1, ly);
  bil_idx(x, sx, lw, x0, x1, lx);
  const float a = low[y0 * lw + x0], b = low[y0 * lw + x1], c = low[y1 * lw + x0], d = low[y1 * lw + x1];
  return (1.f - ly) * ((1.f - lx) * a + lx * b) + ly * ((1.f - lx) * c + lx * d);
}
// ... 518 lines not shown
```

### anyref_amd/csrc/optest.hip

```cpp
#include <algorithm>
#include <string>
#include <vector>

#include "../../include/anyref_hip_ops.h"
#include "kernels.h"

using namespace anyref;

static thread_local std::string g_op_err;
static thread_local std::string g_op_tags;

#define OP_GUARD(...)                                    \
  try {                                                  \
    __VA_ARGS__;                                         \
    hipError_t _e = hipGetLastError();                   \
    if (_e != hipSuccess) {                              \
      g_op_err = std::string("HIP error: ") + hipGetErrorString(_e); \
      return 3;                                          \
    }                                                    \
    return 0;                                            \
  } catch (const std::exception& e) {                    \
    g_op_err = e.what();                                 \
    return 2;                                            \
  }
// ... 214 lines not shown
    else if (t == 2) launch_gemv<f16>(a, (hipStream_t)stream);
    else if (t == 3) launch_gemv<sp16>(a, (hipStream_t)stream);
    else if (t == 4) launch_gemv<sp16h>(a, (hipStream_t)stream);
    else throw std::runtime_error("op_gemv_xn: t = 0 .. 4");
  });
}

int anyref_op_split_roundtrip(int t, void* stream, const float* in, float* out, void* hi_out, int rows, int cols) {
  OP_GUARD({
    if (t != 3 && t != 4) throw std::runtime_error("op_split_roundtrip: t = 3 / 4");
    hipStream_t st = (hipStream_t)stream;
    TmpBuf Ps((size_t)rows * pad64(cols) * 4);
    if (t == 4) launch_convert<sp16h>(in, cols, Ps.p, pad64(cols), rows, cols, st);
    else launch_convert<sp16>(in, cols, Ps.p, pad64(cols), rows, cols, st);
    launch_unsplit(Ps.p, pad64(cols), out, cols, rows, cols, st, t == 4);
    if (hi_out) {
      std::vector<uint16_t> h((size_t)rows * pad64(cols) * 2);
      HIP_TRY(hipStreamSynchronize(st));
      HIP_TRY(hipMemcpy(h.data(), Ps.p, h.size() * 2, hipMemcpyDeviceToHost));
      std::vector<uint16_t> hi((size_t)rows * cols);
      for (int r = 0; r < rows; ++r)
        for (int c = 0; c < cols; ++c) hi[(size_t)r * cols + c] = h[(size_t)r * pad64(cols) * 2 + sp_col(c)];
      HIP_TRY(hipMemcpy(hi_out, hi.data(), hi.size() * 2, hipMemcpyHostToDevice));
    }
  });
}

int anyref_op_rope_table(int S, int hd, float theta, float* out_host) { OP_GUARD(rope_table(S, hd, theta, out_host)); }

int anyref_op_decode_attn(int t, void* stream, const float* qkv, int B, int H, int hd, const int32_t* pos,
                          const float* cs_tab, void* kc, void* vc, int maxS, float scale, float* out, void* q_keep,
                          int force_fallback) {
  OP_GUARD({
    if (t != 0 && t != 1 && t != 2) throw std::runtime_error("op_decode_attn: t = 0 / 1 / 2");
    hipStream_t st = (hipStream_t)stream;
    std::vector<int> h(B);
    HIP_TRY(hipMemcpy(h.data(), pos, (size_t)B * 4, hipMemcpyDeviceToHost));
    for (int& v : h) v += 1;
    TmpBuf kv_len((size_t)B * 4);
    TmpBuf q_tmp((size_t)B * H * hd * 4);
    HIP_TRY(hipMemcpy(kv_len.p, h.data(), (size_t)B * 4, hipMemcpyHostToDevice));
    if (t == 0)
      launch_decode_step_attn<float>(qkv, B, H, hd, pos, (const int*)kv_len.p, cs_tab, q_tmp.p, kc, vc, maxS, scale, out,
                                     q_keep, st, force_fallback != 0);
    else if (t == 2)
      launch_decode_step_attn<f16>(qkv, B, H, hd, pos, (const int*)kv_len.p, cs_tab, q_tmp.p, kc, vc, maxS, scale, out,
                                   q_keep, st, force_fallback != 0);
    else
      launch_decode_step_attn<bf16>(qkv, B, H, hd, pos, (const int*)kv_len.p, cs_tab, q_tmp.p, kc, vc, maxS, scale, out,
                                    q_keep, st, force_fallback != 0);
  });
}

int anyref_op_rope_cache(int t, void* stream, const void* qkv, const float* slab0, const float* slab1, int B, int S, int H,
                         int hd, const int32_t* pos0, const int32_t* lens, const float* cs_tab, void* q_out, void* kc,
                         void* vc, int maxS, void* q_keep) {
  OP_GUARD({
    hipStream_t st = (hipStream_t)stream;
    if (t != 0 && t != 1 && t != 2) throw std::runtime_error("op_rope_cache: t = 0 / 1 / 2");
    if (slab0) {
      if (t == 0) launch_rope_cache_slabs<float>(slab0, slab1, B, S, H, hd, pos0, lens, cs_tab, q_out, kc, vc, maxS, q_keep, st);
      else if (t == 2) launch_rope_cache_slabs<f16>(slab0, slab1, B, S, H, hd, pos0, lens, cs_tab, q_out, kc, vc, maxS, q_keep, st);
      else launch_rope_cache_slabs<bf16>(slab0, slab1, B, S, H, hd, pos0, lens, cs_tab, q_out, kc, vc, maxS, q_keep, st);
    } else if (t == 0)
      launch_rope_cache<float>(qkv, B, S, H, hd, pos0, lens, cs_tab, q_out, kc, vc, maxS, q_keep, st);
    else if (t == 2)
      launch_rope_cache<f16>(qkv, B, S, H, hd, pos0, lens, cs_tab, q_out, kc, vc, maxS, q_keep, st);
    else
      launch_rope_cache<bf16>(qkv, B, S, H, hd, pos0, lens, cs_tab, q_out, kc, vc, maxS, q_keep, st);
  });
}

int anyref_op_argmax(void* stream, const float* x, int M, int N, int ldx, int64_t* out, int32_t* pos, const void* table,
                     int is_bf16, int D, int maxS, float* x_next, int32_t* row_map, int32_t* kvlen) {
  OP_GUARD({
    if (table && (is_bf16 < 0 || is_bf16 > 2)) throw std::runtime_error("op_argmax: table dtype 0 / 1 / 2");
    if (table)
      launch_argmax_next(x, M, N, ldx, out, pos, table, is_bf16, D, maxS, x_next, row_map, kvlen, (hipStream_t)stream);
    else
      launch_argmax(x, M, N, ldx, out, (hipStream_t)stream, pos);
  });
}

int anyref_op_norm(int t, void* stream, const float* x, const float* gain, const float* bias, float* y, int M,
                   int D, float eps, int rms) {
  OP_GUARD({
    NormArgs a;
    a.x = x; a.ldx = D; a.gain = gain; a.bias = bias; a.y = y; a.ldy = D; a.M = M; a.D = D; a.eps = eps;
    a.rms = rms; a.y_f32 = 1;
    if (t == 3 || t == 4) {
      TmpBuf Ys((size_t)M * pad64(D) * 4);
      a.y = Ys.p; a.ldy = pad64(D); a.y_f32 = 0;
      if (t == 4) launch_norm<sp16h>(a, (hipStream_t)stream);
      else launch_norm<sp16>(a, (hipStream_t)stream);
      launch_unsplit(Ys.p, pad64(D), y, D, M, D, (hipStream_t)stream, t == 4);
    } else
    if (t == 0) launch_norm<float>(a, (hipStream_t)stream);
    else if (t == 2) launch_norm<f16>(a, (hipStream_t)stream);
    else launch_norm<bf16>(a, (hipStream_t)stream);
  });
}

int anyref_op_attention(int t, void* stream, const void* q, const void* k, const void* v, void* o, int B, int H,
                        int Sq, int Sk, int hd, float scale, int causal, const int32_t* kv_len,
                        const float* rel_h, const float* rel_w, int kh, int kw) {
  OP_GUARD({
    AttnArgs a;
    a.Q = q; a.K = k; a.V = v; a.O = o;
    a.q_bs = (int64_t)Sq * H * hd; a.q_rs = H * hd; a.q_hs = hd;
    a.k_bs = a.v_bs = (int64_t)Sk * H * hd; a.k_rs = a.v_rs = H * hd; a.k_hs = a.v_hs = hd;
    a.o_bs = (int64_t)Sq * H * hd; a.o_rs = H * hd; a.o_hs = hd;
    a.B = B; a.H = H; a.Sq = Sq; a.Sk = Sk; a.hd = hd; a.scale = scale; a.causal = causal; a.kv_len = kv_len;
    a.rel_h = rel_h; a.rel_w = rel_w; a.kh = kh; a.kw = kw;
    if (t == 3 || t == 4) {
      if ((H * hd) % 64) throw std::runtime_error("op_attention t=3/4: H * hd % 64 != 0");
      TmpBuf Os((size_t)B * Sq * H * hd * 4);
      a.O = Os.p; a.o_split = t == 4 ? 2 : 1; a.sp16 = 1;
      launch_attention<float>(a, (hipStream_t)stream);
      launch_unsplit(Os.p, H * hd, reinterpret_cast<float*>(o), H * hd, B * Sq, H * hd, (hipStream_t)stream, t == 4);
    } else
    if (t == 0) launch_attention<float>(a, (hipStream_t)stream);
    else if (t == 2) launch_attention<f16>(a, (hipStream_t)stream);
    else launch_attention<bf16>(a, (hipStream_t)stream);
  });
}

int anyref_op_attention_tab(int t, void* stream, const void* q, const void* k, const void* v, void* o, int B, int H, int S,
                            int hd, float scale, const void* tab_h, const void* tab_w, int tab_ld, int kh, int kw) {
  OP_GUARD({
    AttnArgs a;
    a.Q = q; a.K = k; a.V = v; a.O = o;
    a.q_bs = a.k_bs = a.v_bs = a.o_bs = (int64_t)S * H * hd;
    a.q_rs = a.k_rs = a.v_rs = a.o_rs = H * hd; a.q_hs = a.k_hs = a.v_hs = a.o_hs = hd;
    a.B = B; a.H = H; a.Sq = S; a.Sk = S; a.hd = hd; a.scale = scale;
    a.rel_tab_h = tab_h; a.rel_tab_w = tab_w; a.rel_tab_ld = tab_ld; a.kh = kh; a.kw = kw;
    if (t == 3 || t == 4) {
      if ((H * hd) % 64) throw std::runtime_error("op_attention_tab t=3/4: H * hd % 64 != 0");
      if (!attention_takes_rel_tables(4, hd, S, S, kh, kw, true)) throw std::runtime_error("op_attention_tab t=3/4: not a window shape");
      TmpBuf Os((size_t)B * S * H * hd * 4);
      a.O = Os.p; a.o_split = t == 4 ? 2 : 1; a.sp16 = 1;
      launch_attention<float>(a, (hipStream_t)stream);
      launch_unsplit(Os.p, H * hd, reinterpret_cast<float*>(o), H * hd, B * S, H * hd, (hipStream_t)stream, t == 4);
    } else
    if (t == 2) launch_attention<f16>(a, (hipStream_t)stream);
    else launch_attention<bf16>(a, (hipStream_t)stream);
  });
}

int anyref_op_gemm_gather(int t, void* stream, const void* A, const int32_t* a_row_map, const void* W, const float* bias,
                          void* C, const float* resid, int M, int N, int K, int c_f32) {
  OP_GUARD({
    GemmArgs a;
    a.A = A; a.lda = K; a.W = W; a.ldw = K; a.bias = bias; a.C = C; a.ldc = N; a.resid = resid; a.ldr = N;
    a.a_row_map = a_row_map; a.M = M; a.N = N; a.K = K; a.c_f32 = c_f32;
    if (t == 2) launch_gemm<f16>(a, (hipStream_t)stream);
    else if (t == 1) launch_gemm<bf16>(a, (hipStream_t)stream);
    else throw std::runtime_error("gemm_gather: 16-bit types only");
  });
}

int anyref_op_attention_relp(int t, void* stream, const void* q, const void* k, const void* v, void* o, int B, int H, int S,
                             int hd, float scale, const float* rel_p, int rel_ld, int kh, int kw) {
  OP_GUARD({
    AttnArgs a;
    a.Q = q; a.K = k; a.V = v; a.O = o;
    a.q_bs = a.k_bs = a.v_bs = a.o_bs = (int64_t)S * H * hd;
// ... 125 lines not shown
```

### include/anyref_hip_ops.h

```cpp
#ifndef ANYREF_HIP_OPS_H
#define ANYREF_HIP_OPS_H
#include <stdint.h>
#ifdef __cplusplus
extern "C" {
#endif

int anyref_op_gemm(int t, void* stream, const void* A, const void* W, const float* bias, void* C,
                   const float* resid, const int32_t* row_map, int M, int N, int K, int act, int c_f32);
int anyref_op_gemv(int t, void* stream, const float* x, const float* gain, float eps, const void* W,
                   const void* W2, const float* bias, float* y, const float* resid, int B, int N, int K, int act);
int anyref_op_gemv_xn(int t, void* stream, const float* x, const float* gain, float eps, const void* W, const void* W2,
                      const float* bias, float* y, const float* resid, int B, int N, int K, int act, float* xn_out,
                      const int32_t* xn_row_map, int xn_ld);
int anyref_op_split_roundtrip(int t, void* stream, const float* in, float* out, void* hi_out, int rows, int cols);
int anyref_op_rope_table(int S, int hd, float theta, float* out_host);
int anyref_op_decode_attn(int t, void* stream, const float* qkv, int B, int H, int hd, const int32_t* pos,
                          const float* cs_tab, void* kc, void* vc, int maxS, float scale, float* out, void* q_keep,
                          int force_fallback);
int anyref_op_rope_cache(int t, void* stream, const void* qkv, const float* slab0, const float* slab1, int B, int S, int H,
                         int hd, const int32_t* pos0, const int32_t* lens, const float* cs_tab, void* q_out, void* kc,
                         void* vc, int maxS, void* q_keep);
int anyref_op_argmax(void* stream, const float* x, int M, int N, int ldx, int64_t* out, int32_t* pos, const void* table,
                     int is_bf16, int D, int maxS, float* x_next, int32_t* row_map, int32_t* kvlen);
int anyref_op_norm(int t, void* stream, const float* x, const float* gain, const float* bias, float* y, int M,
                   int D, float eps, int rms);
int anyref_op_attention(int t, void* stream, const void* q, const void* k, const void* v, void* o, int B, int H,
                        int Sq, int Sk, int hd, float scale, int causal, const int32_t* kv_len,
                        const float* rel_h, const float* rel_w, int kh, int kw);
int anyref_op_rel_pos(int t, void* stream, const void* q, const float* tab_h, const float* tab_w, int B, int H,
                      int size, int hd, float* rel_h, float* rel_w);
int anyref_op_quant_fp8(void* stream, const float* src, int N, int K, uint8_t* q, float* scale);
int anyref_op_gemm_fp8(void* stream, const void* A, const uint8_t* W8, const float* scale, const float* bias, void* C,
                       const float* resid, int M, int N, int K, int act, int c_f32);
int anyref_op_gemv_fp8(void* stream, const float* x, const float* gain, float eps, const uint8_t* W,
                       const uint8_t* W2, const float* scale, const float* scale2, float* y, const float* resid,
                       int B, int N, int K);
int anyref_op_quant_int4(void* stream, const float* src, int N, int K, uint8_t* q, void* scale_bf16);
int anyref_op_dequant_int4(void* stream, const uint8_t* q, const void* scale_bf16, int N, int K, void* out_bf16);
int anyref_op_gemm_int4(void* stream, const void* A, const uint8_t* W4, const void* scale_bf16, const float* bias, void* C,
                        const float* resid, int M, int N, int K, int act, int c_f32, int swiglu);
int anyref_op_gemv_int4(void* stream, const float* x, const float* gain, float eps, const uint8_t* W, const uint8_t* W2,
                        const void* scale_bf16, const void* scale2_bf16, float* y, const float* resid, int B, int N, int K);
int anyref_op_iou_counts(void* stream, const float* logits, const uint8_t* target, int n, int64_t hw,
                         int64_t* counts);
int anyref_op_avs_counts(void* stream, const float* logits, const uint8_t* target, int n, int64_t hw,
                         const float* cuts, int nth, float cut_pred, int64_t* conf, int64_t* hist);
int anyref_op_sam_preprocess(void* stream, const uint8_t* img, int h, int w, int S, const float* mean3,
                             const float* std3, float* out);
int anyref_op_pil_resample_u8(void* stream, const uint8_t* in, int H, int W, int C, uint8_t* tmp, uint8_t* out,
                              int ow, int oh, const int32_t* xbounds, const int32_t* xk, int kx,
                              const int32_t* ybounds, const int32_t* yk, int ky);
int anyref_op_pool_ref_tokens(void* stream, const float* feats, int n, int L, int H, int n_out, float* out);
int anyref_op_clip_finish(void* stream, const uint8_t* img, int ih, int iw, int y0, int x0, int h, int w, int S,
                          const float* mean3, const float* std3, float* out);
int anyref_op_kaldi_fbank(void* stream, const float* wave, int C, int T, int win, int shift, int padded, float preemph,
                          const float* banks, int n_mel, const double* tw, double* scratch, int target_len, float mean,
                          float stdv, float* out);
int anyref_op_attention_tab(int t, void* stream, const void* q, const void* k, const void* v, void* o, int B, int H, int S,
                            int hd, float scale, const void* tab_h, const void* tab_w, int tab_ld, int kh, int kw);
int anyref_op_gemm_gather(int t, void* stream, const void* A, const int32_t* a_row_map, const void* W, const float* bias,
                          void* C, const float* resid, int M, int N, int K, int c_f32);
int anyref_op_attention_relp(int t, void* stream, const void* q, const void* k, const void* v, void* o, int B, int H, int S,
                             int hd, float scale, const float* rel_p, int rel_ld, int kh, int kw);
int anyref_op_postprocess(void* stream, const float* low, int n, int lh, int lw, int S, int rh, int rw, int H,
                          int W, float* out);
const char* anyref_op_last_error(void);

typedef struct anyref_gemm_ex {
  const void* A;
  const void* W;
  const float* bias;
  void* C;
  const float* resid;
  const int32_t* row_map;
  const int32_t* a_row_map;
  const float* norm_gain;
  const float* norm_bias;
  void* norm_out;
  float* slabs_out;
  int64_t sA, sW, sC, sR, sBias;
  int32_t M, N, K, lda, ldw, ldc, ldr, norm_ld;
  int32_t act, c_f32, swiglu_pairs, slabs, max_wg, batch;
  float alpha, norm_eps;
  int32_t norm_done;
} anyref_gemm_ex;
int anyref_op_gemm_ex(int t, void* stream, anyref_gemm_ex* e);

typedef struct anyref_norm_ex {
  const float* x;
  const float* gain;
  const float* bias;
  void* y;
  const int32_t* row_map;
  void* fill_dst;
  const int32_t* fill_rows;
  const float* fill_bias;
  int32_t M, D, ldx, ldy, rms, y_f32, act;
  int32_t fill_ld, fill_n, fill_N;
  int32_t fill_fallback;
  float eps;
  int32_t fill_done;
} anyref_norm_ex;
int anyref_op_norm_ex(int t, void* stream, anyref_norm_ex* e);

typedef struct anyref_attn_ex {
  const void *q, *k, *v;
// ... 16 lines not shown
```

Before: 25.84 images/sec.

## Fuse per-block argmax into LM-head GEMV and write tokens to pinned host memory

The LM-head GEMV now keeps a running argmax per workgroup and stores partial (value, index) pairs. A small finish kernel reduces these, updates pos, row map and kv length, embeds the next token, and writes the token id straight into mapped pinned host memory, so the per-step device-to-host memcpy is no longer needed. The prefill path reads the last hidden rows through an x row map instead of running a separate gather kernel. The aim is to replace a full re-read of the vocab logits and to drop launches and copies from each decode step, in exchange for added kernel complexity and reliance on the ordering of zero-copy host writes.

```diff
diff --git a/anyref_amd/_lib.py b/anyref_amd/_lib.py
--- a/anyref_amd/_lib.py
+++ b/anyref_amd/_lib.py
@@ -128,6 +128,8 @@
     "anyref_op_decode_attn": (_I, [_I, _P, _P, _I, _I, _I, _P, _P, _P, _P, _I, _F, _P, _P, _I]),
     "anyref_op_rope_cache": (_I, [_I, _P, _P, _P, _P, _I, _I, _I, _I, _P, _P, _P, _P, _P, _P, _I, _P]),
     "anyref_op_argmax": (_I, [_P, _P, _I, _I, _I, _P, _P, _P, _I, _I, _I, _P, _P, _P]),
+    "anyref_op_gemv_part": (_I, [_I, _P, _P, _I, _P, _P, _F, _P, _P, _I, _I, _I, _I, _P, _P]),
+    "anyref_op_argmax_finish": (_I, [_P, _P, _P, _I, _P, _P, _P, _I, _I, _I, _P, _P, _P, _P, _I, _I]),
     "anyref_op_norm": (_I, [_I, _P, _P, _P, _P, _P, _I, _I, _F, _I]),
     "anyref_op_attention": (_I, [_I, _P, _P, _P, _P, _P, _I, _I, _I, _I, _I, _F, _I, _P, _P, _P, _I, _I]),
     "anyref_op_attention_tab": (_I, [_I, _P, _P, _P, _P, _P, _I, _I, _I, _I, _F, _P, _P, _I, _I, _I]),
diff --git a/anyref_amd/csrc/common.h b/anyref_amd/csrc/common.h
--- a/anyref_amd/csrc/common.h
+++ b/anyref_amd/csrc/common.h
@@ -313,6 +313,21 @@
   return v;
 }
 
+__device__ __forceinline__ void argmax_take(float v, int i, float& best, int& bi) {
+  const bool vn = __builtin_isnan(v), bn = __builtin_isnan(best);
+  if (vn || bn) {
+    if (vn && (!bn || i < bi)) {
+      best = v;
+      bi = i;
+    }
+    return;
+  }
+  if (v > best || (v == best && i < bi)) {
+    best = v;
+    bi = i;
+  }
+}
+
 #define HIP_TRY(expr)                                                                   \
   do {                                                                                  \
     hipError_t _e = (expr);                                                             \
diff --git a/anyref_amd/csrc/gemv.hip b/anyref_amd/csrc/gemv.hip
--- a/anyref_amd/csrc/gemv.hip
+++ b/anyref_amd/csrc/gemv.hip
@@ -60,7 +60,7 @@
     float4v xv[NB][XV];
 #pragma unroll
     for (int b = 0; b < NB; ++b) {
-      const float* x = a.x + (int64_t)(b0 + (b < nb ? b : 0)) * a.ldx;
+      const float* x = gemv_x_row(a, b0 + (b < nb ? b : 0));
 #pragma unroll
       for (int i = 0; i < XV; ++i) {
         const int k = (tid + i * 512) * 4;
@@ -105,6 +105,7 @@
   for (int r = 0; r < RW; ++r)
 #pragma unroll
     for (int b = 0; b < NB; ++b) acc[r][b] = 0.f;
+  GemvPart part;
   for (int t = 0; t < items; ++t) {
     if (t + 1 < items) load_item(t + 1, wnxt);
     const auto it = wk.item(t);
@@ -162,7 +163,7 @@
         }
       }
     }
-    if (it.last) gemv_finish_group<NB, R, DUAL, W8, PAIR>(a, acc, red2, it.g, it.pass, wk.half, lane, wave, b0, nb);
+    if (it.last) gemv_finish_group<NB, R, DUAL, W8, PAIR>(a, acc, red2, it.g, it.pass, wk.half, lane, wave, b0, nb, part);
     if (t + 1 < items) {
 #pragma unroll
       for (int u = 0; u < UNR; ++u)
@@ -170,6 +171,7 @@
         for (int r = 0; r < RW; ++r) wcur[u][r] = wnxt[u][r];
     }
   }
+  if (a.part_val) gemv_part_store<NB, R>(a, part, lane, wave, b0, nb);
   gemv_stamp_end(a.stamp, st_t, st_cnt, t_begin, lane);
 }
 
@@ -455,6 +457,8 @@
   if (((uintptr_t)a.x & 15) || a.ldx % 4 || a.K % 4 || (a.gain && ((uintptr_t)a.gain & 15)) ||
       (a.xn_out && (((uintptr_t)a.xn_out & 15) || a.xn_ld % 4)))
     throw std::runtime_error("gemv: x / gain / xn_out rows must be 16-byte aligned");
+  if ((a.part_val || a.x_row_map) && a.B > 4)
+    throw std::runtime_error("gemv: partial argmax / x row map: up to 4 rows (the kernels of the 4-row passes)");
   int b0 = 0;
   if constexpr (std::is_same<T, bf16>::value) {
     while (a.B - b0 > 4) {
@@ -468,7 +472,7 @@
 template void launch_gemv<float>(const GemvArgs&, hipStream_t);
 
 void launch_gemv_skinny_f32(const GemvArgs& a, hipStream_t s) {
-  if (a.B < 1 || a.B > 8 || a.K > 4096 || a.K % 4 || a.W2 || a.w_fp8 || a.gain || ((uintptr_t)a.W & 15) ||
+  if (a.B < 1 || a.B > 8 || a.K > 4096 || a.K % 4 || a.W2 || a.w_fp8 || a.gain || a.part_val || a.x_row_map || ((uintptr_t)a.W & 15) ||
       ((uintptr_t)a.x & 15) || a.ldx % 4)
     throw std::runtime_error("gemv_skinny_f32: 1..8 rows, K <= 4096, K % 4 == 0, 16-byte aligned rows");
   const int ngroups = cdiv(a.N, 2);
diff --git a/anyref_amd/csrc/gemv_common.h b/anyref_amd/csrc/gemv_common.h
--- a/anyref_amd/csrc/gemv_common.h
+++ b/anyref_amd/csrc/gemv_common.h
@@ -33,6 +33,10 @@
   }
 };
 
+__device__ __forceinline__ const float* gemv_x_row(const GemvArgs& a, int row) {
+  return a.x + (int64_t)(a.x_row_map ? a.x_row_map[row] : row) * a.ldx;
+}
+
 template <int NB, int XV>
 struct GemvNormStage {
   float4v xr[NB][XV], gr[XV];
@@ -46,7 +50,7 @@
   __device__ __forceinline__ void load_x(const GemvArgs& a, int b0, int nb, int tid) {
 #pragma unroll
     for (int b = 0; b < NB; ++b) {
-      const float* x = a.x + (int64_t)(b0 + (b < nb ? b : 0)) * a.ldx;
+      const float* x = gemv_x_row(a, b0 + (b < nb ? b : 0));
 #pragma unroll
       for (int i = 0; i < XV; ++i) {
         const int k = (tid + i * 512) * 4;
@@ -85,7 +89,7 @@
 }
 
 template <bool DUAL, bool W8>
-__device__ __forceinline__ void gemv_epilogue(const GemvArgs& a, float v, float v2, int n, int row) {
+__device__ __forceinline__ float gemv_epilogue(const GemvArgs& a, float v, float v2, int n, int row) {
   if constexpr (W8) {
     v *= a.wscale[(int64_t)n * a.ws_stride];
     if (DUAL) v2 *= a.wscale2[(int64_t)n * a.ws_stride];
@@ -98,11 +102,46 @@
   const int64_t o = (int64_t)row * a.ldy + n;
   if (a.resid) v += a.resid[o];
   a.y[o] = v;
+  return v;
+}
+
+struct GemvPart {
+  float v = -INFINITY;
+  int i = 0x7fffffff;
+};
+template <int NB, int R>
+__device__ __forceinline__ void gemv_part_store(const GemvArgs& a, GemvPart p, int lane, int wave, int b0, int nb) {
+  __shared__ float pv[8][NB];
+  __shared__ int pi[8][NB];
+  if constexpr (R == 2) {
+    const float v = __shfl_xor(p.v, NB, 64);
+    const int i = __shfl_xor(p.i, NB, 64);
+    argmax_take(v, i, p.v, p.i);
+  }
+  if (lane < NB) {
+    pv[wave][lane] = p.v;
+    pi[wave][lane] = p.i;
+  }
+  __syncthreads();
+  const int b = wave * 64 + lane;
+  if (b < nb) {
+    GemvPart q;
+#pragma unroll
+    for (int w = 0; w < 8; ++w) argmax_take(pv[w][b], pi[w][b], q.v, q.i);
+    float* val = a.part_val + (size_t)(b0 + b) * GEMV_PART_SLOTS;
+    int* idx = a.part_idx + (size_t)(b0 + b) * GEMV_PART_SLOTS;
+    val[blockIdx.x] = q.v;
+    idx[blockIdx.x] = q.i;
+    for (unsigned s = blockIdx.x + gridDim.x; s < (unsigned)GEMV_PART_SLOTS; s += gridDim.x) {
+      val[s] = -INFINITY;
+      idx[s] = 0x7fffffff;
+    }
+  }
 }
 
 template <int NB, int R, bool DUAL, bool W8, bool PAIR>
 __device__ __forceinline__ void gemv_finish_group(const GemvArgs& a, float (&acc)[2][NB], float (&red2)[2][4][2][NB], int g,
-                                                  int pass, int half, int lane, int wave, int b0, int nb) {
+                                                  int pass, int half, int lane, int wave, int b0, int nb, GemvPart& part) {
   constexpr int RW = 2;
   const int n0 = g * R;
 #pragma unroll
@@ -136,7 +175,10 @@
           v = acc[rr][bb];
           v2 = DUAL ? acc[RW - 1][bb] : 0.f;
         }
-    if (n < a.N && b < nb) gemv_epilogue<DUAL, W8>(a, v, v2, n, b0 + b);
+    if (n < a.N && b < nb) {
+      const float y = gemv_epilogue<DUAL, W8>(a, v, v2, n, b0 + b);
+      if (a.part_val) argmax_take(y, n, part.v, part.i);
+    }
   }
 #pragma unroll
   for (int r = 0; r < RW; ++r)
@@ -208,6 +250,8 @@
   GemvArgs a = a_in;
   if (lds > 150 * 1024) throw std::runtime_error(std::string(name) + ": K too large for the LDS activation stage");
   const GemvPlan p = gemv_plan(a, lds);
+  if (a.part_val && (!a.part_idx || p.grid > GEMV_PART_SLOTS))
+    throw std::runtime_error(std::string(name) + ": partial argmax needs both arrays and a grid of at most GEMV_PART_SLOTS");
   auto go = [&](auto xpt_t) {
     char tag[40];
     snprintf(tag, sizeof(tag), "gemv_%s%s_x%d", kind, a.W2 ? "_swiglu" : "", decltype(xpt_t)::value);
diff --git a/anyref_amd/csrc/gemv_int4.hip b/anyref_amd/csrc/gemv_int4.hip
--- a/anyref_amd/csrc/gemv_int4.hip
+++ b/anyref_amd/csrc/gemv_int4.hip
@@ -182,6 +182,7 @@
   for (int r = 0; r < RW; ++r)
 #pragma unroll
     for (int b = 0; b < NB; ++b) acc[r][b] = 0.f;
+  GemvPart part;
   for (int t = 0; t < items; ++t) {
     if (t + 1 < items) load_item(t + 1, wnxt, snxt);
     const auto it = wk.item(t);
@@ -224,7 +225,7 @@
         }
       }
     }
-    if (it.last) gemv_finish_group<NB, R, DUAL, false, PAIR>(a, acc, red2, it.g, it.pass, wk.half, lane, wave, b0, nb);
+    if (it.last) gemv_finish_group<NB, R, DUAL, false, PAIR>(a, acc, red2, it.g, it.pass, wk.half, lane, wave, b0, nb, part);
     if (t + 1 < items) {
 #pragma unroll
       for (int u = 0; u < UNR; ++u)
@@ -235,6 +236,7 @@
         }
     }
   }
+  if (a.part_val) gemv_part_store<NB, R>(a, part, lane, wave, b0, nb);
   gemv_stamp_end(a.stamp, st_t, st_cnt, t_begin, lane);
 }
 
@@ -256,6 +258,7 @@
   if (((uintptr_t)a.x & 15) || a.ldx % 4 || (a.gain && ((uintptr_t)a.gain & 15)) ||
       (a.xn_out && (((uintptr_t)a.xn_out & 15) || a.xn_ld % 4)))
     throw std::runtime_error("gemv_int4: x / gain / xn_out rows must be 16-byte aligned");
+  if ((a.part_val || a.x_row_map) && a.B > 4) throw std::runtime_error("gemv_int4: partial argmax / x row map: up to 4 rows");
   gemv_passes<4>(0, a.B, [&](auto nb_t, int b0, int nb) { gemv_int4_dispatch<decltype(nb_t)::value>(a, b0, nb, s); });
 }
 
diff --git a/anyref_amd/csrc/kernels.h b/anyref_amd/csrc/kernels.h
--- a/anyref_amd/csrc/kernels.h
+++ b/anyref_amd/csrc/kernels.h
@@ -162,7 +162,11 @@
   int xn_ld = 0;
   StampArgs stamp;
   int grid = 0;
-};
+  float* part_val = nullptr;
+  int* part_idx = nullptr;
+  const int* x_row_map = nullptr;
+};
+constexpr int GEMV_PART_SLOTS = 512;
 template <typename T>
 void launch_gemv(const GemvArgs& a, hipStream_t s);
 void launch_gemv_skinny_f32(const GemvArgs& a, hipStream_t s);
@@ -292,6 +296,9 @@
 void launch_argmax(const float* x, int M, int N, int ldx, int64_t* out, hipStream_t s, int* bump = nullptr);
 void launch_argmax_next(const float* x, int M, int N, int ldx, int64_t* out, int* pos, const void* table, int dtype,
                         int D, int maxS, float* x_next, int* row_map, int* kvlen, hipStream_t s);
+void launch_argmax_finish(const float* part_val, const int* part_idx, int M, int64_t* out, int* pos, const void* table,
+                          int dtype, int D, int maxS, float* x_next, int* row_map, int* kvlen, int64_t* host_tok,
+                          int host_stride, hipStream_t s, bool tie_high = false);
 template <typename T>
 void launch_upscale1(const float* tmp, int n, int g, int C, const float* ln_g, const float* ln_b, float eps,
                      void* out, hipStream_t s);
diff --git a/anyref_amd/csrc/model.hip b/anyref_amd/csrc/model.hip
--- a/anyref_amd/csrc/model.hip
+++ b/anyref_amd/csrc/model.hip
@@ -416,6 +416,7 @@
   hipEvent_t ev_fork_ = nullptr, ev_sam_ = nullptr;
   bool sam_forked_ = false;
   void decode_step_graph(hipStream_t s, int B, bool keep_q, bool corun = false);
+  void llm_greedy_tail(hipStream_t s, int B, GemvArgs& h);
   hipStream_t cap_stream_ = nullptr;
   std::map<int, hipGraphExec_t> decode_graphs_;
   int splice_inputs(hipStream_t s, const int64_t* input_ids, const int32_t* lens, int B, int Lmax,
@@ -460,6 +461,11 @@
   int *lens_dev_ = nullptr, *slen_dev_ = nullptr, *pos_dev_ = nullptr, *kvlen_dev_ = nullptr, *rowmap_dev_ = nullptr,
       *idx_a_ = nullptr, *idx_b_ = nullptr;
   int64_t* next_host_ = nullptr;
+  float* part_val_ = nullptr;
+  int* part_idx_ = nullptr;
+  int64_t* next_host_dev_ = nullptr;
+  bool seam_argmax_ = !(getenv("ANYREF_SEAM_ARGMAX") && atoi(getenv("ANYREF_SEAM_ARGMAX")) == 0);
+  bool greedy_seam(int B) const { return seam_argmax_ && B <= 4; }
   hipEvent_t ev_tok_[2] = {nullptr, nullptr};
   int* stage_ = nullptr;
   int *stage_first_ = nullptr, *stage_extra_ = nullptr, *stage_seg_ = nullptr, *stage_kl_ = nullptr;
@@ -801,6 +807,9 @@
     idx_a_ = talloc<int>((size_t)MB * std::max(c.max_seg, 64));
     idx_b_ = talloc<int>((size_t)MB * std::max(c.max_seg, 64));
     HIP_TRY(hipHostMalloc((void**)&next_host_, sizeof(int64_t) * MB * 2));
+    HIP_TRY(hipHostGetDevicePointer((void**)&next_host_dev_, next_host_, 0));
+    part_val_ = talloc<float>((size_t)std::min(MB, 4) * GEMV_PART_SLOTS);
+    part_idx_ = talloc<int>((size_t)std::min(MB, 4) * GEMV_PART_SLOTS);
     for (auto& e : ev_tok_) HIP_TRY(hipEventCreateWithFlags(&e, hipEventDisableTiming));
     {
       const int n_first = 3 * MB, n_extra_max = 2 * MB * std::max(c.max_seg, 64), n_seg = 2 * MB * c.max_seg;
@@ -1355,9 +1364,22 @@
   h.x = d_x_; h.ldx = H; h.gain = llm_norm_.g; h.eps = c.llm_rms_eps; gemv_w(h, lm_head_); h.y = l_logits_;
   h.ldy = c.llm_vocab; h.B = B; h.N = c.llm_vocab; h.K = H;
   h.xn_out = hidden_all_; h.xn_row_map = rowmap_dev_; h.xn_ld = H;
+  llm_greedy_tail(s, B, h);
+}
+
+template <typename T, typename TS>
+void Model<T, TS>::llm_greedy_tail(hipStream_t s, int B, GemvArgs& h) {
+  const anyref_config& c = cfg;
+  if (greedy_seam(B)) {
+    h.part_val = part_val_; h.part_idx = part_idx_;
+    launch_gemv<T>(h, s);
+    launch_argmax_finish(part_val_, part_idx_, B, next_dev_, pos_dev_, emb_table_, kEmbDtype, c.llm_dim, c.llm_max_seq, d_x_,
+                         rowmap_dev_, kvlen_dev_, next_host_dev_, c.max_batch, s);
+    return;
+  }
   launch_gemv<T>(h, s);
-  launch_argmax_next(l_logits_, B, c.llm_vocab, c.llm_vocab, next_dev_, pos_dev_, emb_table_, kEmbDtype, H, S, d_x_,
-                     rowmap_dev_, kvlen_dev_, s);
+  launch_argmax_next(l_logits_, B, c.llm_vocab, c.llm_vocab, next_dev_, pos_dev_, emb_table_, kEmbDtype, c.llm_dim,
+                     c.llm_max_seq, d_x_, rowmap_dev_, kvlen_dev_, s);
 }
 
 template <typename T, typename TS>
@@ -1811,6 +1833,7 @@
   if (max_new_tokens < 1) throw std::runtime_error("max_new_tokens must be >= 1");
   const int H = c.llm_dim, S = c.llm_max_seq, n_img = clip_n_;
   const bool keep_q = c.rephrase_weight > 0.f;
+  const bool seam = greedy_seam(B);
 
   SamJoinGuard<Model<T, TS>> join_guard{this, s};
   const int nblk = (int)sam_blocks_.size();
@@ -1857,20 +1880,23 @@
     int *bb = stage_first_, *pp = stage_first_ + B, *sl = stage_first_ + 2 * B;
     for (int b = 0; b < B; ++b) {
       bb[b] = b;
-      pp[b] = slen[b] - 1;
+      pp[b] = seam ? b * S + slen[b] - 1 : slen[b] - 1;
       sl[b] = slen[b] - 1;
     }
-    HIP_TRY(hipMemcpyAsync(idx_a_, bb, B * 4, hipMemcpyHostToDevice, s));
+    if (!seam) HIP_TRY(hipMemcpyAsync(idx_a_, bb, B * 4, hipMemcpyHostToDevice, s));
     HIP_TRY(hipMemcpyAsync(idx_b_, pp, B * 4, hipMemcpyHostToDevice, s));
     HIP_TRY(hipMemcpyAsync(pos_dev_, sl, B * 4, hipMemcpyHostToDevice, s));
     }
-    launch_gather_rows(hidden_all_, S, H, idx_a_, idx_b_, B, l_xlast_, s);
     GemvArgs h;
-    h.x = l_xlast_; h.ldx = H; gemv_w(h, lm_head_); h.y = l_logits_; h.ldy = c.llm_vocab; h.B = B; h.N = c.llm_vocab;
+    if (seam) {
+      h.x = hidden_all_; h.x_row_map = idx_b_;
+    } else {
+      launch_gather_rows(hidden_all_, S, H, idx_a_, idx_b_, B, l_xlast_, s);
+      h.x = l_xlast_;
+    }
+    h.ldx = H; gemv_w(h, lm_head_); h.y = l_logits_; h.ldy = c.llm_vocab; h.B = B; h.N = c.llm_vocab;
     h.K = H;
-    launch_gemv<T>(h, s);
-    launch_argmax_next(l_logits_, B, c.llm_vocab, c.llm_vocab, next_dev_, pos_dev_, emb_table_, kEmbDtype, H, S, d_x_,
-                       rowmap_dev_, kvlen_dev_, s);
+    llm_greedy_tail(s, B, h);
   }
   std::vector<std::vector<int64_t>> gen(B);
   std::vector<char> fin(B, 0);
@@ -1888,8 +1914,9 @@
   };
   for (int step = 0; step < max_new_tokens; ++step) {
     int64_t* tok = next_host_ + (size_t)(step & 1) * c.max_batch;
+    auto tok_of = [&](int b) { return seam ? next_host_[(size_t)((slen[b] + step) & 1) * c.max_batch + b] : tok[b]; };
     const bool last = step == max_new_tokens - 1;
-    HIP_TRY(hipMemcpyAsync(tok, next_dev_, B * 8, hipMemcpyDeviceToHost, s));
+    if (!seam) HIP_TRY(hipMemcpyAsync(tok, next_dev_, B * 8, hipMemcpyDeviceToHost, s));
     HIP_TRY(hipEventRecord(ev_tok_[step & 1], s));
     if (ahead && !last) {
       decode_step_graph(s, B, keep_q, corun_step());
@@ -1899,9 +1926,10 @@
     bool all = true;
     for (int b = 0; b < B; ++b) {
       if (!fin[b]) {
-        gen[b].push_back(tok[b]);
-        if (eos_token_id >= 0 && tok[b] == eos_token_id) fin[b] = 1;
-        if (early && !early_stop_ && tok[b] >= c.seg_lo && tok[b] <= c.seg_hi)
+        const int64_t tk = tok_of(b);
+        gen[b].push_back(tk);
+        if (eos_token_id >= 0 && tk == eos_token_id) fin[b] = 1;
+        if (early && !early_stop_ && tk >= c.seg_lo && tk <= c.seg_hi)
           early_seg(ev_tok_[step & 1], slen[0] + step - 1, resized_hw, orig_hw, out_masks, out_masks_cap, out_low);
       }
       all = all && fin[b];
diff --git a/anyref_amd/csrc/ops.hip b/anyref_amd/csrc/ops.hip
--- a/anyref_amd/csrc/ops.hip
+++ b/anyref_amd/csrc/ops.hip
@@ -979,20 +979,6 @@
 template void launch_swiglu<bf16>(const void*, int, int, void*, hipStream_t);
 template void launch_swiglu<f16>(const void*, int, int, void*, hipStream_t);
 
-__device__ __forceinline__ void argmax_take(float v, int i, float& best, int& bi) {
-  const bool vn = __builtin_isnan(v), bn = __builtin_isnan(best);
-  if (vn || bn) {
-    if (vn && (!bn || i < bi)) {
-      best = v;
-      bi = i;
-    }
-    return;
-  }
-  if (v > best || (v == best && i < bi)) {
-    best = v;
-    bi = i;
-  }
-}
 struct ArgmaxNext {
   const void* table = nullptr;
   int dtype = 0, D = 0, maxS = 0;
@@ -1072,6 +1058,67 @@
   ArgmaxNext nx;
   nx.table = table; nx.dtype = dtype; nx.D = D; nx.maxS = maxS; nx.x = x_next; nx.row_map = row_map; nx.kvlen = kvlen;
   hipLaunchKernelGGL(argmax_kernel, dim3(M), dim3(1024), 0, s, x, N, ldx, out, pos, nx);
+}
+
+template <bool TIE_HIGH>
+__global__ __launch_bounds__(256) void argmax_finish_kernel(const float* __restrict__ pv, const int* __restrict__ pi,
+                                                            int64_t* __restrict__ out, int* __restrict__ pos, ArgmaxNext nx,
+                                                            int64_t* __restrict__ host_tok, int host_stride) {
+  constexpr int NT = 256, U = GEMV_PART_SLOTS / 64;
+  const int b = blockIdx.x, tid = threadIdx.x;
+  __shared__ int si;
+  if (tid < 64) {
+    float v[U];
+    int idx[U];
+#pragma unroll
+    for (int u = 0; u < U; ++u) {
+      v[u] = pv[(size_t)b * GEMV_PART_SLOTS + u * 64 + tid];
+      idx[u] = pi[(size_t)b * GEMV_PART_SLOTS + u * 64 + tid];
+    }
+    float best = -INFINITY;
+    int bi = 0x7fffffff;
+    auto take = [&](float w, int i) {
+      if (TIE_HIGH && w == best && bi != 0x7fffffff) {
+        if (i != 0x7fffffff && i > bi) bi = i;
+      } else {
+        argmax_take(w, i, best, bi);
+      }
+    };
+#pragma unroll
+    for (int u = 0; u < U; ++u) take(v[u], idx[u]);
+#pragma unroll
+    for (int o = 32; o > 0; o >>= 1) {
+      const float w = __shfl_xor(best, o, 64);
+      const int i = __shfl_xor(bi, o, 64);
+      take(w, i);
+    }
+    if (tid == 0) {
+      out[b] = bi;
+      si = bi;
+      const int p = pos[b] + 1;
+      pos[b] = p;
+      nx.row_map[b] = b * nx.maxS + p;
+      nx.kvlen[b] = p + 1;
+      if (host_tok) host_tok[(size_t)(p & 1) * host_stride + b] = bi;
+    }
+  }
+  __syncthreads();
+  table_row_to_f32(nx.table, nx.dtype, si, nx.D, nx.x + (int64_t)b * nx.D, tid, NT);
+}
+void launch_argmax_finish(const float* part_val, const int* part_idx, int M, int64_t* out, int* pos, const void* table,
+                          int dtype, int D, int maxS, float* x_next, int* row_map, int* kvlen, int64_t* host_tok,
+                          int host_stride, hipStream_t s, bool tie_high) {
+  if (M <= 0) return;
+  if (!part_val || !part_idx || !out || !pos || !table || !x_next || !row_map || !kvlen || (host_tok && host_stride < M))
+    throw std::runtime_error("argmax_finish: partial pairs, pos, table and the next step's arrays are all required");
+  ArgmaxNext nx;
+  nx.table = table; nx.dtype = dtype; nx.D = D; nx.maxS = maxS; nx.x = x_next; nx.row_map = row_map; nx.kvlen = kvlen;
+  if (tie_high)
+    hipLaunchKernelGGL(argmax_finish_kernel<true>, dim3(M), dim3(256), 0, s, part_val, part_idx, out, pos, nx, host_tok,
+                       host_stride);
+  else
+    hipLaunchKernelGGL(argmax_finish_kernel<false>, dim3(M), dim3(256), 0, s, part_val, part_idx, out, pos, nx, host_tok,
+                       host_stride);
 }
 
 template <typename T>
diff --git a/anyref_amd/csrc/optest.hip b/anyref_amd/csrc/optest.hip
--- a/anyref_amd/csrc/optest.hip
+++ b/anyref_amd/csrc/optest.hip
@@ -320,6 +320,26 @@
   });
 }
 
+int anyref_op_gemv_part(int t, void* stream, const float* x, int ldx, const int32_t* x_row_map, const float* gain, float eps,
+                        const void* W, float* y, int B, int N, int K, int grid, float* part_val, int32_t* part_idx) {
+  OP_GUARD({
+    GemvArgs a;
+    a.x = x; a.ldx = ldx; a.x_row_map = x_row_map; a.gain = gain; a.eps = eps; a.W = W; a.y = y; a.ldy = N; a.B = B; a.N = N;
+    a.K = K; a.grid = grid; a.part_val = part_val; a.part_idx = part_idx;
+    by_type(t, [&](auto T0) { launch_gemv<decltype(T0)>(a, (hipStream_t)stream); });
+  });
+}
+
+int anyref_op_argmax_finish(void* stream, const float* part_val, const int32_t* part_idx, int M, int64_t* out, int32_t* pos,
+                            const void* table, int dtype, int D, int maxS, float* x_next, int32_t* row_map, int32_t* kvlen,
+                            int64_t* host_tok, int host_stride, int tie_high) {
+  OP_GUARD({
+    if (dtype < 0 || dtype > 2) throw std::runtime_error("op_argmax_finish: table dtype 0 / 1 / 2");
+    launch_argmax_finish(part_val, part_idx, M, out, pos, table, dtype, D, maxS, x_next, row_map, kvlen, host_tok, host_stride,
+                         (hipStream_t)stream, tie_high != 0);
+  });
+}
+
 int anyref_op_norm(int t, void* stream, const float* x, const float* gain, const float* bias, float* y, int M,
                    int D, float eps, int rms) {
   OP_GUARD({
diff --git a/include/anyref_hip_ops.h b/include/anyref_hip_ops.h
--- a/include/anyref_hip_ops.h
+++ b/include/anyref_hip_ops.h
@@ -22,6 +22,11 @@
                          void* vc, int maxS, void* q_keep);
 int anyref_op_argmax(void* stream, const float* x, int M, int N, int ldx, int64_t* out, int32_t* pos, const void* table,
                      int is_bf16, int D, int maxS, float* x_next, int32_t* row_map, int32_t* kvlen);
+int anyref_op_gemv_part(int t, void* stream, const float* x, int ldx, const int32_t* x_row_map, const float* gain, float eps,
+                        const void* W, float* y, int B, int N, int K, int grid, float* part_val, int32_t* part_idx);
+int anyref_op_argmax_finish(void* stream, const float* part_val, const int32_t* part_idx, int M, int64_t* out, int32_t* pos,
+                            const void* table, int dtype, int D, int maxS, float* x_next, int32_t* row_map, int32_t* kvlen,
+                            int64_t* host_tok, int host_stride, int tie_high);
 int anyref_op_norm(int t, void* stream, const float* x, const float* gain, const float* bias, float* y, int M,
                    int D, float eps, int rms);
 int anyref_op_attention(int t, void* stream, const void* q, const void* k, const void* v, void* o, int B, int H,
```

Result: no change. 25.82 images/sec (median of 3 runs) (-0.1%).
